# wangkenpu/rsrgan

Measured on AMD Instinct MI355X. Metric: GAN train frames/sec (G+D step), 257-dim LPS->40-dim MFCC, higher is better.
Workload: dtype f32

## Files before the change

### rsrgan_amd/csrc/kernels.h

```cpp
#pragma once
#include <hip/hip_runtime.h>
#include <stdint.h>

#include "switches.h"

namespace rsr {

constexpr int MAXJ = 8;

struct Place { int x0, nx, sb, se, nb, w; };
constexpr int JOBMAP_MAX = 768;
struct JobMap { int valid; unsigned char job[JOBMAP_MAX]; };
struct PlanItem { int ncol, nrow; double cost; int mult; };
int plan_places(int n, const PlanItem* items, Place* out);

enum { DYN_G_LR = 0, DYN_D_LR = 1, DYN_LAMBDA = 2, DYN_D_REAL = 3, DYN_D_FAKE = 4, DYN_L2 = 5, DYN_CLIP = 6,
       DYN_B1 = 7, DYN_B2 = 8, DYN_EPS = 9, DYN_EMA = 10, DYN_ADAM_LRT = 11, DYN_ADAM_LRT_D = 12, DYN_COUNT = 16 };

struct FwdGateJob {
  const float* x;
  const float* KxT;
  const float* m;
  const float* KhT;
  const float* Wsw;
// ... 100 lines not shown
  unsigned long long* gran;
  unsigned* ctl;
  float forget_bias;
  const float* dout_top;
  int ld_dout;
  float* dy;
  const float* fc_w;
  float* dtop;
  int ld_dy, ld_fcw, ld_dtop, fc_P;
  const float* fc_b;
  const float* noise;
  int xd_Ns, xd_row0;
  int Ns, row0;
  int nrt;
  float* dw_ws;
  unsigned* dw_flag;
  size_t dw_stride;
};
int dpersist_dw_grid(int nl, int N);
size_t dpersist_dw_stride(const DPersistArgs& a);
size_t dpersist_dw_flag_bytes(int nl, int N, int T);
bool dpersist_dw_supported(const DPersistArgs& a);
size_t dpersist_granule_bytes(int nl, int N, int T);
int dpersist_trail_grid(int nl, int N);
size_t dpersist_trail_lds_bytes();
bool dpersist_trail_supported(const DPersistArgs& a);
bool dpersist_supported(const DPersistArgs& a);
int dpersist_grid(int nl, int N);
size_t dpersist_lds_bytes();
void launch_dlstm_fwd(const DPersistArgs& a, hipStream_t s);
void launch_dlstm_fwd_t(const DPersistArgs& a, hipStream_t s);
void launch_dlstm_bwd(const DPersistArgs& a, hipStream_t s);
constexpr int GP_MAXL = 4;
constexpr int GP_ROWS = 32;
constexpr int GP_THREADS = 768;
struct GPersistLayer {
  const float *KxT, *KhT;
  const float *bias, *wi, *wf, *wo, *Wp;
  float *gates, *c, *h, *mst, *out;
  const float* in;
  float* dmt;
  int I, P, ldI, ldP, ldH;
  float* res_out;
};
struct GPersistArgs {
  GPersistLayer L[GP_MAXL];
  int nl, N, T, H;
  int NT, NC;
  const int* len;
  unsigned long long *gran1, *gran2;
  unsigned* ctl;
  float forget_bias;
  unsigned long long* gran3;
  const float* dout_top;
  int ld_dout;
  float* din0;
  int ld_din0;
  int res;
  int tags;
  int dout_trail;
  int fwd_trail;
  int ngl, grp0;
  int nrt;
  int sched;
  int carry;
};
constexpr int GP_TMAX = 2046;
bool gpersist_plan(GPersistArgs& a);
void gpersist_arm_bytes(void* p, size_t bytes, hipStream_t s);
extern thread_local int g_gemm_workers;
int gpersist_grid(const GPersistArgs& a);
int gpersist_dt_grid(const GPersistArgs& a, const DPersistArgs& d);
void launch_glstm_fwd_dt(const GPersistArgs& a, const DPersistArgs& d, hipStream_t s);
size_t dpersist_fwdt_lds_bytes();
void launch_glstm_bwd_dt(const GPersistArgs& a, const DPersistArgs& d, hipStream_t s);
size_t gpersist_lds_bytes();
int device_cu_count();
bool resident_probe(int grid, int threads, size_t lds_bytes);
size_t gpersist_gran1_bytes(const GPersistArgs& a);
size_t gpersist_gran2_bytes(const GPersistArgs& a);
size_t gpersist_gran3_bytes(const GPersistArgs& a);
void gpersist_arm(const GPersistArgs& a, hipStream_t s);
void launch_glstm_fwd(const GPersistArgs& a, hipStream_t s);
bool gpersist_np_plan(GPersistArgs& a, int nt_force = 0);
size_t gpersist_np_gran2_bytes(const GPersistArgs& a);
size_t gpersist_np_lds_bytes();
void launch_glstm_np_fwd(const GPersistArgs& a, hipStream_t s);
size_t gpersist_np_gran1_bytes(const GPersistArgs& a);
size_t gpersist_np_gran3_bytes(const GPersistArgs& a);
void gpersist_np_arm(const GPersistArgs& a, hipStream_t s);
void launch_glstm_np_bwd(const GPersistArgs& a, hipStream_t s);
void launch_glstm_bwd(const GPersistArgs& a, hipStream_t s);
extern long long g_chain_launches;
void launch_floor_chain(float* a, float* b, int n, int mode, hipStream_t s);

struct GemmRowMap { int rows_per; long long outer; long long inner; };
void launch_gemm_mapped(const float* A, int lda, const GemmRowMap& ma, const float* A2, int lda2, int M1, bool a_kc, const float* B, int ldb,
                        bool b_kc, float* C, int ldc, int M, int N, int K, const float* bias, int act, float alpha,
                        bool accumulate, hipStream_t s, float* ws, size_t ws_floats);
constexpr int GEMM16_MAXB = 4;
struct Gemm16Batch { const float* A[GEMM16_MAXB]; const float* A2[GEMM16_MAXB]; const float* B[GEMM16_MAXB]; float* C[GEMM16_MAXB]; int n; };
void launch_gemm16_batch(const Gemm16Batch& bt, int lda, int lda2, int M1, int ldb, int ldc, int M, int N, int K, bool accumulate,
                         hipStream_t s, float* ws, size_t ws_floats);
void launch_gemm2(const float* A, int lda, const float* A2, int lda2, int M1, bool a_kc, const float* B, int ldb, bool b_kc,
                  float* C, int ldc, int M, int N, int K, const float* bias, int act, float alpha, bool accumulate,
                  hipStream_t s, float* ws, size_t ws_floats);
constexpr int GEMM_MAXB = 4;
bool launch_gemm_batch(int nb, const float* const* A, int lda, const float* const* A2, int lda2, int M1, const float* const* B, int ldb,
                       float* const* C, int ldc, int M, int N, int K, bool accumulate, hipStream_t s, float* ws, size_t ws_floats);
void launch_gemm(const float* A, int lda, bool a_kc, const float* B, int ldb, bool b_kc,
                 float* C, int ldc, int M, int N, int K,
                 const float* bias, int act, float alpha, bool accumulate, hipStream_t s,
                 float* splitk_ws = nullptr, size_t splitk_ws_floats = 0);

struct StagePack { const float* src; float* dst; int D, ld; };
struct StageCopy { const void* src; void* dst; int n; };
struct StageJobs { StagePack pack[2]; StageCopy copy[4]; int B, T; int Bt; };
void launch_stage_inputs(const StageJobs& j, hipStream_t s);
void launch_pack_tm(const float* src_bm, float* dst_tm, int B, int T, int D, int ld, hipStream_t s);
void launch_unpack_bm(const float* src_tm, int ld, float* dst_bm, int B, int T, int D, hipStream_t s, int Bt = 0);
void launch_build_d_input(const float* lab_tm, const float* y_tm, const float* noise_r, const float* noise_f,
                          float* xd, int B, int T, int D, int ld, bool with_real, hipStream_t s);
void launch_add_noise_rows(const float* src_tm, const float* noise, float* dst, int B, int T, int D, int ld,
                           int Ns, int row0, hipStream_t s);
void launch_transpose(const float* src, int lds, float* dst, int ldd, int R, int C, hipStream_t s);
void launch_fill(float* p, size_t n, float v, hipStream_t s);
struct SwizzleJob { const float* src; float* dst; int ld, gates, H, C, c0, K1, I, P, kx, nct, nkb, blk_base; };
struct SwizzleList { int n; SwizzleJob j[24]; };
void launch_swizzle_many(SwizzleList& sl, hipStream_t s);
inline size_t swizzle_floats(int nct, int nkb) { return (size_t)nct * nkb * 256; }
struct TransposeJob { const float* src; float* dst; int lds, ldd, R, C, blk_base; };
struct TransposeList { int n; TransposeJob j[16]; };
void launch_transpose_many(TransposeList& tl, hipStream_t s);
size_t conv_prep_floats(int S, int fw, int C);
void launch_conv_prep(const float* F, int ldf_src, int S, int fw, int Cin, int Cout, bool flip, float* Ft, hipStream_t s);
bool conv_fwd_supported(int C, int N, int S, int W, int fw);
void launch_conv_fwd(const float* in, int ldc_in, int C, const float* Ft, const float* bias, bool relu, float* out, int ldc_out, int N,
                     int R, int S, int W, int fw, hipStream_t s,
                     const float* mask = nullptr );
bool conv_wgrad_supported(int C, int N, int S, int W, int fw);
size_t conv_wgrad_ws_floats(int C, int R, int S, int W, int fw);
void launch_conv_wgrad(const float* in, int ldc_in, int C, const float* d, int ldc_d, int N, float* dW, int ldw, float* ws, int R, int S,
                       int W, int fw, hipStream_t s,
                       float* db = nullptr );
void launch_im2col(const float* src, size_t row_stride, int ldc, int C, int S, int W, int kh, int kw, float* col, int ldk, size_t M,
                   hipStream_t s);
void launch_expand_c4(const float* src, int ld_src, int n, float* dst, size_t rows, hipStream_t s);
void launch_col2im(const float* dcol, int ldk, int C, int S, int W, int kh, int kw, float* dst, int ldc, size_t M, hipStream_t s);
struct GStateLayer { float *c, *mst; int H, P, ldP, off; };
struct GStateArgs { GStateLayer L[GP_MAXL]; int nl, SF, rows, dir; float* state; size_t slot; const int* mask; };
void launch_gstate(const GStateArgs& a, hipStream_t s);
struct ZeroList { int n; float* p[32]; unsigned len[32]; };
void launch_zero_many(const ZeroList& zl, hipStream_t s);
struct ColsumsBatch { const float* dz[4]; const float* cprev[4]; const float* ccur[4]; float* db[4]; float* dwi[4]; float* dwf[4]; float* dwo[4]; int n; };
void launch_lstm_colsums_batch(const ColsumsBatch& bt, int rows, int H, float* scratch, hipStream_t s);
void launch_lstm_colsums(const float* dz, const float* cprev, const float* ccur, float* db, float* dwi, float* dwf, float* dwo,
                         int rows, int H, float* scratch , hipStream_t s);
void launch_lrelu_bwd(const float* hval, float* d, size_t rows, int cols, int ld, float alpha, hipStream_t s);
void launch_dropout_fwd(float* y, size_t rows, int cols, int ld, unsigned long long key, unsigned thr, float keep, hipStream_t s);
void launch_dropout_bwd(const float* y, float* d, size_t rows, int cols, int ld, float keep, hipStream_t s);
void launch_colsum_tall(const float* a, int lda, float* out, int rows, int cols, float* scratch, size_t scratch_floats, hipStream_t s);

struct BnVars {
  float *beta, *gamma;
  float *mm, *mv, *rm, *rmw, *rs, *rsw;
};
constexpr int BN_STAT_ROWS = 6;
void launch_bn_forward(const float* z, int ldz, float* y, int ldy, int rows, int cols, const BnVars& v, float* stat, int ldc, bool training,
                       bool relu, float* scratch, size_t scratch_floats, hipStream_t s, int calls = 1);
void launch_bn_backward(float* dy, int ldd, const float* y, int ldy, const float* z, int ldz, int rows, int cols, const float* stat, int ldc,
                        float* dbeta, float* dgamma, bool accumulate, bool relu, float* sums, float* scratch, size_t scratch_floats,
                        hipStream_t s, int calls = 1);
void launch_bn_commit(int cols, const BnVars& v, const float* stat, int ldc, int times, hipStream_t s);
struct BnCommit { BnVars v; const float* stat; int cols, ldc, times0, times1; };
struct BnCommitList { int n; BnCommit e[24]; };
void launch_bn_commit_many(const BnCommitList& cl, hipStream_t s);
void launch_colsum(const float* a, int lda, const float* b, int ldb, float* out, int rows, int cols,
                   float* scratch , hipStream_t s);

constexpr int DH_MAXR = 64;
struct DHeadArgs {
  const float* top; int ldt; const float* w; int ldw; const float* b;
  float* logits; int ldl; float* dlogits; float* dout; int ldo; float* gw; float* gb;
  int T, Nd, n_real, dR; const float* t_real; const float* t_fake; float* loss3; float* part; int want_grads, want_wgrads;
  int Bp, Bt;
};
void launch_dhead(const DHeadArgs& a, hipStream_t s);
void launch_lsgan(const float* logits, int ldl, float* dlogits, int T, int Nd, int n_real,
                  const float* target_real, const float* target_fake, float* loss3, hipStream_t s,
                  bool clip_on = false, float clip_lo = 0.f, float clip_hi = 0.f, int Bp = 0, int Bt = 0);
void launch_build_joint(const float* x, int ldx, int off, int dim, const float* tail, int ldt, int Dt, float* joint, int ldj,
                        int row0, int R, hipStream_t s);
void launch_slice_cols(const float* src, int lds, int off, float* dst, int ldd, int R, int C, hipStream_t s);
void launch_mse(const float* y, const float* lab, int ld, float* dy, int rows, int D, const float* lambda,
                bool accumulate, float* loss_out, float* scratch , hipStream_t s, int Bp = 0, int Bt = 0);
void launch_g_total(float* l4 , const float* lambda, hipStream_t s);
void launch_copy_f(const float* src, float* dst, int n, hipStream_t s);

struct ChunkTable {
  const int* tensor;
  const int* off;
  const int* len;
  const int* t_first;
  const int* t_count;
  const int* t_l2;
  int n_chunks, n_tensors;
};
void launch_sumsq(const float* g, const ChunkTable& ct, float* partial, hipStream_t s);
void launch_dw_reduce(const float* ws, size_t stride, int ntiles, const long long* src, float* g, const ChunkTable& ct, float* partial, hipStream_t s);
void launch_l2(const float* w, float* g, const ChunkTable& ct, const float* l2_scale, float* partial, hipStream_t s);
void launch_l2_total(const float* partial, int n_chunks, const float* l2_scale, float* out, hipStream_t s);
void launch_apply_sgd(float* w, const float* g, float* ema, const ChunkTable& ct, const float* partial,
                      const float* dyn, hipStream_t s);
void launch_apply_adam(float* w, const float* g, float* m, float* v, float* ema, const ChunkTable& ct,
                       const float* partial, const float* dyn, hipStream_t s, int lrt_slot = DYN_ADAM_LRT);
void launch_adam_tick(float* dyn, int* t, double b1, double b2, hipStream_t s, int lr_slot = DYN_G_LR, int lrt_slot = DYN_ADAM_LRT);
void launch_pad_copy(const float* dense, float* padded, int rows, int cols, int ld, bool to_padded, hipStream_t s);

}
```

### rsrgan_amd/csrc/kernels.hip

```cpp
#include <algorithm>
#include <cstdlib>

#include "kernels.h"

namespace rsr {

typedef float f32x4 __attribute__((ext_vector_type(4)));

__device__ __forceinline__ float sigmoid_(float x) { return 1.0f / (1.0f + expf(-x)); }

#ifdef RSR_TRACE
__device__ unsigned long long g_trace[8192 * 16];
#define TR_BEGIN() do { if (threadIdx.x == 0 && blockIdx.x < 8192) { unsigned long long* t_ = g_trace + (size_t)blockIdx.x * 16; \
    t_[0] = __builtin_amdgcn_s_memrealtime(); t_[1] = __builtin_amdgcn_s_memtime(); \
    t_[14] = __builtin_amdgcn_s_getreg(4 | (0 << 6) | (31 << 11)); t_[15] = __builtin_amdgcn_s_getreg(20 | (0 << 6) | (3 << 11)); \
    for (int i_ = 2; i_ < 14; ++i_) t_[i_] = 0; } } while (0)
#define TR_ID(ptr) do { if (threadIdx.x == 0 && blockIdx.x < 8192) g_trace[(size_t)blockIdx.x * 16 + 12] = (unsigned long long)(size_t)(ptr); } while (0)
#define TR(i) do { if (threadIdx.x == 0 && blockIdx.x < 8192) g_trace[(size_t)blockIdx.x * 16 + (i)] = __builtin_amdgcn_s_memtime(); } while (0)
#define TR_END() do { if (threadIdx.x == 0 && blockIdx.x < 8192) { g_trace[(size_t)blockIdx.x * 16 + 9] = __builtin_amdgcn_s_memtime(); \
    g_trace[(size_t)blockIdx.x * 16 + 13] = __builtin_amdgcn_s_memrealtime(); } } while (0)
#else
#define TR_BEGIN() do { } while (0)
#define TR_ID(ptr) do { } while (0)
#define TR(i) do { } while (0)
#define TR_END() do { } while (0)
#endif

template <typename T>
__device__ __forceinline__ T* as_global(T* p) { return (T*)(__attribute__((address_space(1))) T*)(unsigned long long)p; }
#define RSR_G(f) J.f = as_global(J.f);
__device__ __forceinline__ unsigned long long splitmix64(unsigned long long x) {
  x += 0x9E3779B97F4A7C15ull;
  x = (x ^ (x >> 30)) * 0xBF58476D1CE4E5B9ull;
  x = (x ^ (x >> 27)) * 0x94D049BB133111EBull;
  return x ^ (x >> 31);
}
__device__ __forceinline__ unsigned long long drop_key(const DropSpec& d) {
  return splitmix64(splitmix64(d.seed ^ (*d.ctr * 0xD1342543DE82EF95ull)) + d.tag);
}
__device__ __forceinline__ bool drop_on(unsigned long long key, size_t idx, unsigned thr) { return (unsigned)(splitmix64(key + idx) >> 40) < thr; }
__device__ __forceinline__ void globalize(FwdGateJob& J) {
  RSR_G(x) RSR_G(KxT) RSR_G(m) RSR_G(KhT) RSR_G(Wsw) RSR_G(zx) RSR_G(bias) RSR_G(wf) RSR_G(wi) RSR_G(wo) RSR_G(c_prev) RSR_G(c_out) RSR_G(gates)
  RSR_G(h) RSR_G(len) RSR_G(np_m_out) RSR_G(np_out) RSR_G(np_res_in) RSR_G(np_res_out)
}
__device__ __forceinline__ void globalize(FwdProjJob& J) {
  RSR_G(h) RSR_G(WpT) RSR_G(WpT_sw) RSR_G(m_prev) RSR_G(m_out) RSR_G(out) RSR_G(res_in) RSR_G(res_out) RSR_G(len) RSR_G(bias) RSR_G(noise)
  J.drop.ctr = as_global(J.drop.ctr);
}
__device__ __forceinline__ void globalize(BwdAJob& J) {
  RSR_G(dout) RSR_G(dmst) RSR_G(Wp) RSR_G(Wp_sw) RSR_G(dmt) RSR_G(gates) RSR_G(c_prev) RSR_G(c_cur) RSR_G(wf) RSR_G(wi) RSR_G(wo) RSR_G(dc) RSR_G(len)
  J.drop.ctr = as_global(J.drop.ctr);
}
__device__ __forceinline__ void globalize(BwdBJob& J) { RSR_G(dz) RSR_G(K) RSR_G(Ksw) RSR_G(dx) RSR_G(dmst) RSR_G(len) RSR_G(ws) }
#undef RSR_G
template <typename JobT, int OFF>
__device__ __forceinline__ JobT pick_job(const JobT* j, const int& n_ref, const JobMap& map, int bid, int& lb) {
  constexpr int ND = (int)(sizeof(JobT) / 4);
  static_assert(sizeof(JobT) % 4 == 0 && ND <= 64 && OFF + 5 < ND, "job record must fit one dword per lane");
  const int lane = threadIdx.x & 63;
  const int li = lane < ND ? lane : 0;
  unsigned v[MAXJ];
#pragma unroll
  for (int q = 0; q < MAXJ; ++q) v[q] = reinterpret_cast<const unsigned*>(j + q)[li];
  const int x = bid & 7, sr = bid >> 3;
  unsigned vs = v[0];
  lb = -1;
  if (map.valid) {
    const int ji = map.job[min(bid, JOBMAP_MAX - 1)];
#pragma unroll
    for (int q = 1; q < MAXJ; ++q) vs = ji == q ? v[q] : vs;
    const int x0 = __builtin_amdgcn_readlane((int)vs, OFF), nx = __builtin_amdgcn_readlane((int)vs, OFF + 1);
    const int sb = __builtin_amdgcn_readlane((int)vs, OFF + 2);
    lb = ji == 0xFF ? -1 : (sr - sb) * nx + ((x - x0) & 7);
  } else {
    const int n = n_ref;
#pragma unroll
    for (int q = 0; q < MAXJ; ++q) {
      const int x0 = __builtin_amdgcn_readlane((int)v[q], OFF), nx = __builtin_amdgcn_readlane((int)v[q], OFF + 1);
      const int sb = __builtin_amdgcn_readlane((int)v[q], OFF + 2), se = __builtin_amdgcn_readlane((int)v[q], OFF + 3);
      const int nb = __builtin_amdgcn_readlane((int)v[q], OFF + 4);
      const int k = (x - x0) & 7;
      const int l = (sr - sb) * nx + k;
      const bool take = q < n && k < nx && sr >= sb && sr < se && l < nb;
      vs = take ? v[q] : vs;
      lb = take ? l : lb;
    }
  }
  union U { JobT j; unsigned d[ND]; __device__ U() {} } u;
#pragma unroll
  for (int i = 0; i < ND; ++i) u.d[i] = (unsigned)__builtin_amdgcn_readlane((int)vs, i);
  globalize(u.j);
  return u.j;
}
#define RSR_PICK(JobT, field, lb) pick_job<JobT, (int)(__builtin_offsetof(JobT, field) / 4)>(jobs.j, jobs.n, jobs.map, bid, lb)
#define RSR_PICK_M(JobT, field, mapf, lb) pick_job<JobT, (int)(__builtin_offsetof(JobT, field) / 4)>(jobs.j, jobs.n, jobs.mapf, bid, lb)

template <typename JobT>
__device__ __forceinline__ JobT load_job(const JobT* p) {
  constexpr int ND = (int)(sizeof(JobT) / 4);
  static_assert(sizeof(JobT) % 4 == 0 && ND <= 64, "job record must fit one dword per lane");
  const int lane = threadIdx.x & 63;
  const unsigned v = reinterpret_cast<const unsigned*>(p)[lane < ND ? lane : 0];
  union U { JobT j; unsigned d[ND]; __device__ U() {} } u;
#pragma unroll
  for (int i = 0; i < ND; ++i) u.d[i] = (unsigned)__builtin_amdgcn_readlane((int)v, i);
  globalize(u.j);
  return u.j;
}

__device__ __forceinline__ bool tile_of_block(int lb, int nblk_c, const Place& pl, int& cb, int& rb) {
  if (lb < 0) return false;
  rb = lb / pl.w;
  cb = lb - rb * pl.w;
  return cb < nblk_c;
}

template <int RT>
struct Seg {
  const float* a[RT];
  const float* w;
  const float* wt;
  int ld;
  int nkb;
  bool wok;
};

template <int RT, int CH, bool TILED>
__device__ __forceinline__ void load_chunk(float4 (&av)[CH][RT], float4 (&bv)[CH], const Seg<RT>& s, int j0, int je, int q) {
#pragma unroll
  for (int c = 0; c < CH; ++c) {
    const int j = j0 + c, jc = min(j, s.nkb - 1);
    const int k = jc * 16 + 4 * q, kc = min(k, s.ld - 4);
    const float4 b = TILED ? *reinterpret_cast<const float4*>(s.wt + (size_t)jc * 256) : *reinterpret_cast<const float4*>(s.w + kc);
    const bool ok = (j < je) && (k < s.ld) && (TILED || s.wok);
    bv[c] = make_float4(ok ? b.x : 0.f, ok ? b.y : 0.f, ok ? b.z : 0.f, ok ? b.w : 0.f);
#pragma unroll
    for (int i = 0; i < RT; ++i) av[c][i] = *reinterpret_cast<const float4*>(s.a[i] + kc);
  }
}
template <int RT, int CH>
__device__ __forceinline__ void mma_chunk(f32x4 (&acc)[RT], const float4 (&av)[CH][RT], const float4 (&bv)[CH]) {
#pragma unroll
  for (int c = 0; c < CH; ++c) {
#pragma unroll
    for (int i = 0; i < RT; ++i) acc[i] = __builtin_amdgcn_mfma_f32_16x16x4f32(av[c][i].x, bv[c].x, acc[i], 0, 0, 0);
#pragma unroll
    for (int i = 0; i < RT; ++i) acc[i] = __builtin_amdgcn_mfma_f32_16x16x4f32(av[c][i].y, bv[c].y, acc[i], 0, 0, 0);
#pragma unroll
    for (int i = 0; i < RT; ++i) acc[i] = __builtin_amdgcn_mfma_f32_16x16x4f32(av[c][i].z, bv[c].z, acc[i], 0, 0, 0);
#pragma unroll
    for (int i = 0; i < RT; ++i) acc[i] = __builtin_amdgcn_mfma_f32_16x16x4f32(av[c][i].w, bv[c].w, acc[i], 0, 0, 0);
  }
}
// ... 1014 lines not shown
    else *o = v[0];
  }
}
void launch_im2col(const float* src, size_t row_stride, int ldc, int C, int S, int W, int kh, int kw, float* col, int ldk, size_t M,
                   hipStream_t s) {
  if (C % 4 == 0 && ldc % 4 == 0) {
    const size_t total = M * (size_t)(ldk / 4);
    hipLaunchKernelGGL(k_im2col<4>, dim3((unsigned)std::min<size_t>((total + 255) / 256, 1u << 20)), dim3(256), 0, s, src, row_stride, ldc, C,
                       S, W, kh, kw, col, ldk, M);
  } else {
    const size_t total = M * (size_t)ldk;
    hipLaunchKernelGGL(k_im2col<1>, dim3((unsigned)std::min<size_t>((total + 255) / 256, 1u << 20)), dim3(256), 0, s, src, row_stride, ldc, C,
                       S, W, kh, kw, col, ldk, M);
  }
}
__global__ __launch_bounds__(256) void k_col2im(const float* __restrict__ dcol, int ldk, int C, int S, int W, int kh, int kw,
                                                float* __restrict__ dst, int ldc, size_t M) {
  const int nv = ldc / 4;
  const size_t total = M * (size_t)nv;
  const int pt = (kh - 1) / 2, pl = (kw - 1) / 2;
  for (size_t i = (size_t)blockIdx.x * blockDim.x + threadIdx.x; i < total; i += (size_t)gridDim.x * blockDim.x) {
    const size_t p = i / nv;
    const int c = (int)(i - p * nv) * 4;
    const int w = (int)(p % W);
    const size_t rh = p / W;
    const int h = (int)(rh % S);
    float4 acc = make_float4(0.f, 0.f, 0.f, 0.f);
    if (c < C) {
      for (int dh = 0; dh < kh; ++dh) {
        const int ho = h - dh + pt;
        if (ho < 0 || ho >= S) continue;
        for (int dw = 0; dw < kw; ++dw) {
          const int wo = w - dw + pl;
          if (wo < 0 || wo >= W) continue;
          const size_t po = (rh - h + ho) * W + wo;
          const float4 t = *reinterpret_cast<const float4*>(dcol + po * ldk + (size_t)(dh * kw + dw) * C + c);
          acc.x += t.x; acc.y += t.y; acc.z += t.z; acc.w += t.w;
        }
      }
    }
    *reinterpret_cast<float4*>(dst + p * ldc + c) = acc;
  }
}
__global__ void k_expand_c4(const float* __restrict__ src, int ld_src, int n, float4* __restrict__ dst, size_t total) {
  for (size_t i = (size_t)blockIdx.x * blockDim.x + threadIdx.x; i < total; i += (size_t)gridDim.x * blockDim.x) {
    const size_t r = i / n;
    dst[i] = make_float4(src[r * ld_src + (i - r * n)], 0.f, 0.f, 0.f);
  }
}
void launch_expand_c4(const float* src, int ld_src, int n, float* dst, size_t rows, hipStream_t s) {
  const size_t total = rows * (size_t)n;
  hipLaunchKernelGGL(k_expand_c4, dim3((unsigned)std::min<size_t>((total + 255) / 256, 1u << 20)), dim3(256), 0, s, src, ld_src, n,
                     reinterpret_cast<float4*>(dst), total);
}
void launch_col2im(const float* dcol, int ldk, int C, int S, int W, int kh, int kw, float* dst, int ldc, size_t M, hipStream_t s) {
  const size_t total = M * (size_t)(ldc / 4);
  hipLaunchKernelGGL(k_col2im, dim3((unsigned)std::min<size_t>((total + 255) / 256, 1u << 20)), dim3(256), 0, s, dcol, ldk, C, S, W, kh, kw,
                     dst, ldc, M);
}

__global__ void k_gstate(GStateArgs a) {
  const int row = blockIdx.x, tid = threadIdx.x;
  float* st = a.state + (size_t)row * a.SF;
  if (a.dir == 2) {
    if (a.mask && a.mask[row] == 0) return;
    for (int i = tid; i < a.SF; i += blockDim.x) st[i] = 0.f;
    return;
  }
  for (int l = 0; l < a.nl; ++l) {
    const GStateLayer L = a.L[l];
    float* c = L.c + (a.slot + row) * L.H;
    float* m = L.mst + (a.slot + row) * L.ldP;
    float* sc = st + L.off;
    float* sm = sc + L.H;
    if (a.dir == 0) {
      for (int i = tid; i < L.H; i += blockDim.x) c[i] = sc[i];
      for (int i = tid; i < L.ldP; i += blockDim.x) m[i] = i < L.P ? sm[i] : 0.f;
    } else {
      for (int i = tid; i < L.H; i += blockDim.x) sc[i] = c[i];
      for (int i = tid; i < L.P; i += blockDim.x) sm[i] = m[i];
    }
  }
}
void launch_gstate(const GStateArgs& a, hipStream_t s) {
  if (a.rows <= 0) return;
  hipLaunchKernelGGL(k_gstate, dim3(a.rows), dim3(256), 0, s, a);
}

__global__ void k_zero_many(ZeroList zl) {
  const int j = blockIdx.y;
  if (j >= zl.n) return;
  float* p = zl.p[j];
  const size_t n = zl.len[j];
  for (size_t i = (size_t)blockIdx.x * blockDim.x + threadIdx.x; i < n; i += (size_t)gridDim.x * blockDim.x) p[i] = 0.f;
}
void launch_zero_many(const ZeroList& zl, hipStream_t s) {
  if (zl.n == 0) return;
  hipLaunchKernelGGL(k_zero_many, dim3(32, zl.n), dim3(256), 0, s, zl);
}

__global__ void k_fill(float* p, size_t n, float v) {
  for (size_t i = (size_t)blockIdx.x * blockDim.x + threadIdx.x; i < n; i += (size_t)gridDim.x * blockDim.x) p[i] = v;
}
void launch_fill(float* p, size_t n, float v, hipStream_t s) {
  if (n == 0) return;
  const int blocks = (int)min((size_t)2048, (n + 255) / 256);
  hipLaunchKernelGGL(k_fill, dim3(blocks), dim3(256), 0, s, p, n, v);
}

__global__ void k_lrelu_bwd(const float* __restrict__ hval, float* __restrict__ d, size_t rows, int cols, int ld, float alpha) {
  const size_t total = rows * (size_t)cols;
  for (size_t i = (size_t)blockIdx.x * blockDim.x + threadIdx.x; i < total; i += (size_t)gridDim.x * blockDim.x) {
    const size_t r = i / cols; const int c = (int)(i % cols);
    const size_t o = r * ld + c;
    if (!(hval[o] > 0.f)) d[o] *= alpha;
  }
}
void launch_lrelu_bwd(const float* hval, float* d, size_t rows, int cols, int ld, float alpha, hipStream_t s) {
  const size_t total = rows * cols;
  const int blocks = (int)min((size_t)2048, (total + 255) / 256);
  hipLaunchKernelGGL(k_lrelu_bwd, dim3(blocks), dim3(256), 0, s, hval, d, rows, cols, ld, alpha);
}

__global__ void k_drop_tick(unsigned long long* ctr) { if (threadIdx.x == 0) *ctr += 1ull; }
void launch_drop_tick(unsigned long long* ctr, hipStream_t s) { hipLaunchKernelGGL(k_drop_tick, dim3(1), dim3(64), 0, s, ctr); }
__global__ __launch_bounds__(256) void k_dropout_fwd(float* __restrict__ y, size_t rows, int cols, int ld, unsigned long long key, unsigned thr,
                                                     float keep) {
  const size_t n = rows * (size_t)cols;
  for (size_t i = (size_t)blockIdx.x * 256 + threadIdx.x; i < n; i += (size_t)gridDim.x * 256) {
    const size_t r = i / cols;
    float* p = y + r * ld + (i - r * cols);
    const bool on = (unsigned)(splitmix64(key + i) >> 40) < thr;
    *p = on ? *p / keep : 0.f;
  }
}
void launch_dropout_fwd(float* y, size_t rows, int cols, int ld, unsigned long long key, unsigned thr, float keep, hipStream_t s) {
  const size_t n = rows * (size_t)cols;
  if (n == 0) return;
  hipLaunchKernelGGL(k_dropout_fwd, dim3((unsigned)std::min<size_t>((n + 255) / 256, 8192)), dim3(256), 0, s, y, rows, cols, ld, key, thr, keep);
}
__global__ __launch_bounds__(256) void k_dropout_bwd(const float* __restrict__ y, float* __restrict__ d, size_t rows, int cols, int ld, float keep) {
  const size_t n = rows * (size_t)cols;
  for (size_t i = (size_t)blockIdx.x * 256 + threadIdx.x; i < n; i += (size_t)gridDim.x * 256) {
    const size_t r = i / cols, o = r * ld + (i - r * cols);
    d[o] = y[o] > 0.f ? d[o] / keep : 0.f;
  }
}
void launch_dropout_bwd(const float* y, float* d, size_t rows, int cols, int ld, float keep, hipStream_t s) {
  const size_t n = rows * (size_t)cols;
  if (n == 0) return;
  hipLaunchKernelGGL(k_dropout_bwd, dim3((unsigned)std::min<size_t>((n + 255) / 256, 8192)), dim3(256), 0, s, y, d, rows, cols, ld, keep);
}

constexpr int CS_SLICES = 64;
__global__ __launch_bounds__(256) void k_colsum1(const float* __restrict__ a, int lda, const float* __restrict__ b, int ldb,
                                                 float* __restrict__ scratch, int rows, int cols) {
  __shared__ float red[4][64];
  const int c = blockIdx.x * 64 + (threadIdx.x & 63), rl = threadIdx.x >> 6;
  const int per = (rows + CS_SLICES - 1) / CS_SLICES;
  const int rbeg = blockIdx.y * per, rend = min(rows, rbeg + per);
  float s = 0.f;
  if (c < cols) {
    for (int r = rbeg + rl; r < rend; r += 4) {
      const float v = a[(size_t)r * lda + c];
      s += b ? v * b[(size_t)r * ldb + c] : v;
    }
  }
  red[rl][threadIdx.x & 63] = s;
  __syncthreads();
  if (rl == 0 && c < cols)
    scratch[(size_t)blockIdx.y * cols + c] = ((red[0][threadIdx.x] + red[1][threadIdx.x]) + red[2][threadIdx.x]) + red[3][threadIdx.x];
}
__global__ void k_colsum2(const float* __restrict__ scratch, float* __restrict__ out, int cols) {
  const int c = blockIdx.x * blockDim.x + threadIdx.x;
  if (c >= cols) return;
  float s = 0.f;
  for (int i = 0; i < CS_SLICES; ++i) s += scratch[(size_t)i * cols + c];
  out[c] = s;
}
__global__ __launch_bounds__(256) void k_colsum1_n(const float* __restrict__ a, int lda, float* __restrict__ scratch, int rows, int cols,
                                                   int per) {
  __shared__ float red[4][64];
  const int c = blockIdx.x * 64 + (threadIdx.x & 63), rl = threadIdx.x >> 6;
  const int rbeg = blockIdx.y * per, rend = min(rows, rbeg + per);
  float s = 0.f;
  if (c < cols) {
#pragma unroll 4
    for (int r = rbeg + rl; r < rend; r += 4) s += a[(size_t)r * lda + c];
  }
  red[rl][threadIdx.x & 63] = s;
  __syncthreads();
  if (rl == 0 && c < cols)
    scratch[(size_t)blockIdx.y * cols + c] = ((red[0][threadIdx.x] + red[1][threadIdx.x]) + red[2][threadIdx.x]) + red[3][threadIdx.x];
}
__global__ __launch_bounds__(256) void k_colsum2_n(const float* __restrict__ scratch, float* __restrict__ out, int cols, int slices) {
  __shared__ float red[4][64];
  const int c = blockIdx.x * 64 + (threadIdx.x & 63), g = threadIdx.x >> 6;
  float s = 0.f;
  if (c < cols) {
#pragma unroll 4
    for (int i = g; i < slices; i += 4) s += scratch[(size_t)i * cols + c];
  }
  red[g][threadIdx.x & 63] = s;
  __syncthreads();
  if (g == 0 && c < cols) out[c] = ((red[0][threadIdx.x] + red[1][threadIdx.x]) + red[2][threadIdx.x]) + red[3][threadIdx.x];
}
void launch_colsum_tall(const float* a, int lda, float* out, int rows, int cols, float* scratch, size_t scratch_floats, hipStream_t s) {
  int slices = (int)std::min<size_t>(512, scratch_floats / (size_t)std::max(cols, 1));
  slices = std::max(1, std::min(slices, (rows + 63) / 64));
  const int per = (rows + slices - 1) / slices;
  slices = (rows + per - 1) / per;
  hipLaunchKernelGGL(k_colsum1_n, dim3((cols + 63) / 64, slices), dim3(256), 0, s, a, lda, scratch, rows, cols, per);
  hipLaunchKernelGGL(k_colsum2_n, dim3((cols + 63) / 64), dim3(256), 0, s, scratch, out, cols, slices);
}

__global__ __launch_bounds__(256) void k_lstm_colsums1(const float* __restrict__ dz, const float* __restrict__ cprev,
                                                       const float* __restrict__ ccur, float* __restrict__ scratch, int rows, int H) {
  __shared__ float red[7][4][64];
  const int c = blockIdx.x * 64 + (threadIdx.x & 63), rl = threadIdx.x >> 6;
  const int per = (rows + CS_SLICES - 1) / CS_SLICES;
  const int rbeg = blockIdx.y * per, rend = min(rows, rbeg + per);
  float s[7] = {0.f, 0.f, 0.f, 0.f, 0.f, 0.f, 0.f};
  if (c < H) {
#pragma unroll 4
    for (int r = rbeg + rl; r < rend; r += 4) {
      const float* z = dz + (size_t)r * 4 * H + c;
      const float di = z[0], dj = z[H], df = z[2 * H], d_o = z[3 * H];
      const float cp = cprev[(size_t)r * H + c], cc = ccur[(size_t)r * H + c];
      s[0] += di; s[1] += dj; s[2] += df; s[3] += d_o; s[4] += di * cp; s[5] += df * cp; s[6] += d_o * cc;
    }
  }
#pragma unroll
  for (int k = 0; k < 7; ++k) red[k][rl][threadIdx.x & 63] = s[k];
  __syncthreads();
  if (rl == 0 && c < H) {
    const int x = threadIdx.x;
#pragma unroll
    for (int k = 0; k < 7; ++k)
      scratch[((size_t)blockIdx.y * 7 + k) * H + c] = ((red[k][0][x] + red[k][1][x]) + red[k][2][x]) + red[k][3][x];
  }
}
__global__ void k_lstm_colsums2(const float* __restrict__ scratch, float* __restrict__ db, float* __restrict__ dwi,
                                float* __restrict__ dwf, float* __restrict__ dwo, int H) {
  const int c = blockIdx.x * blockDim.x + threadIdx.x;
  if (c >= H) return;
  float s[7] = {0.f, 0.f, 0.f, 0.f, 0.f, 0.f, 0.f};
#pragma unroll 8
  for (int i = 0; i < CS_SLICES; ++i)
#pragma unroll
    for (int k = 0; k < 7; ++k) s[k] += scratch[((size_t)i * 7 + k) * H + c];
  db[c] = s[0]; db[H + c] = s[1]; db[2 * H + c] = s[2]; db[3 * H + c] = s[3];
  dwi[c] = s[4]; dwf[c] = s[5]; dwo[c] = s[6];
}
__global__ __launch_bounds__(256) void k_lstm_colsums1_b(const ColsumsBatch bt, float* __restrict__ scratch, int rows, int H) {
  __shared__ float red[7][4][64];
  const int p = blockIdx.z;
  const float* __restrict__ dz = bt.dz[p]; const float* __restrict__ cprev = bt.cprev[p]; const float* __restrict__ ccur = bt.ccur[p];
  scratch += (size_t)p * CS_SLICES * 7 * H;
  const int c = blockIdx.x * 64 + (threadIdx.x & 63), rl = threadIdx.x >> 6;
  const int per = (rows + CS_SLICES - 1) / CS_SLICES;
  const int rbeg = blockIdx.y * per, rend = min(rows, rbeg + per);
  float s[7] = {0.f, 0.f, 0.f, 0.f, 0.f, 0.f, 0.f};
  if (c < H) {
#pragma unroll 4
    for (int r = rbeg + rl; r < rend; r += 4) {
      const float* z = dz + (size_t)r * 4 * H + c;
      const float di = z[0], dj = z[H], df = z[2 * H], d_o = z[3 * H];
      const float cp = cprev[(size_t)r * H + c], cc = ccur[(size_t)r * H + c];
      s[0] += di; s[1] += dj; s[2] += df; s[3] += d_o; s[4] += di * cp; s[5] += df * cp; s[6] += d_o * cc;
    }
  }
#pragma unroll
  for (int k = 0; k < 7; ++k) red[k][rl][threadIdx.x & 63] = s[k];
  __syncthreads();
  if (rl == 0 && c < H) {
    const int x = threadIdx.x;
#pragma unroll
    for (int k = 0; k < 7; ++k)
      scratch[((size_t)blockIdx.y * 7 + k) * H + c] = ((red[k][0][x] + red[k][1][x]) + red[k][2][x]) + red[k][3][x];
  }
}
__global__ void k_lstm_colsums2_b(const float* __restrict__ scratch, const ColsumsBatch bt, int H) {
  const int p = blockIdx.y;
  scratch += (size_t)p * CS_SLICES * 7 * H;
  const int c = blockIdx.x * blockDim.x + threadIdx.x;
  if (c >= H) return;
  float s[7] = {0.f, 0.f, 0.f, 0.f, 0.f, 0.f, 0.f};
#pragma unroll 8
  for (int i = 0; i < CS_SLICES; ++i)
#pragma unroll
    for (int k = 0; k < 7; ++k) s[k] += scratch[((size_t)i * 7 + k) * H + c];
  float* db = bt.db[p];
  db[c] = s[0]; db[H + c] = s[1]; db[2 * H + c] = s[2]; db[3 * H + c] = s[3];
  bt.dwi[p][c] = s[4]; bt.dwf[p][c] = s[5]; bt.dwo[p][c] = s[6];
}
void launch_lstm_colsums_batch(const ColsumsBatch& bt, int rows, int H, float* scratch, hipStream_t s) {
  hipLaunchKernelGGL(k_lstm_colsums1_b, dim3((H + 63) / 64, CS_SLICES, bt.n), dim3(256), 0, s, bt, scratch, rows, H);
  hipLaunchKernelGGL(k_lstm_colsums2_b, dim3((H + 255) / 256, bt.n), dim3(256), 0, s, scratch, bt, H);
}
void launch_lstm_colsums(const float* dz, const float* cprev, const float* ccur, float* db, float* dwi, float* dwf, float* dwo,
                         int rows, int H, float* scratch, hipStream_t s) {
  hipLaunchKernelGGL(k_lstm_colsums1, dim3((H + 63) / 64, CS_SLICES), dim3(256), 0, s, dz, cprev, ccur, scratch, rows, H);
  hipLaunchKernelGGL(k_lstm_colsums2, dim3((H + 255) / 256), dim3(256), 0, s, scratch, db, dwi, dwf, dwo, H);
}

void launch_colsum(const float* a, int lda, const float* b, int ldb, float* out, int rows, int cols, float* scratch, hipStream_t s) {
  hipLaunchKernelGGL(k_colsum1, dim3((cols + 63) / 64, CS_SLICES), dim3(256), 0, s, a, lda, b, ldb, scratch, rows, cols);
  hipLaunchKernelGGL(k_colsum2, dim3((cols + 255) / 256), dim3(256), 0, s, scratch, out, cols);
}

__device__ __forceinline__ float block_sum_1024(float v, float* red) {
  for (int o = 32; o > 0; o >>= 1) v += __shfl_down(v, o, 64);
  const int w = threadIdx.x >> 6;
  if ((threadIdx.x & 63) == 0) red[w] = v;
  __syncthreads();
  float s = 0.f;
  const int nw = (blockDim.x + 63) >> 6;
  for (int i = 0; i < nw; ++i) s += red[i];
  __syncthreads();
  return s;
}

__global__ __launch_bounds__(1024) void k_lsgan(const float* __restrict__ logits, int ldl, float* __restrict__ dlogits,
                                                int T, int Nd, int n_real, const float* __restrict__ t_real,
                                                const float* __restrict__ t_fake, float* __restrict__ loss3,
                                                int clip_on, float clip_lo, float clip_hi, int Bp, int Bt) {
  __shared__ float red[16];
  const int rows = T * Nd;
  const float tr = *t_real, tf = *t_fake;
  const int nr_ = Bp > 0 ? n_real / Bp * Bt : n_real, nf_ = Bp > 0 ? (Nd - n_real) / Bp * Bt : Nd - n_real;
  const float cr = (float)T * (float)nr_, cf = (float)T * (float)nf_;
  float sr = 0.f, sf = 0.f;
  for (int r = threadIdx.x; r < rows; r += blockDim.x) {
    const bool real = (r % Nd) < n_real;
    const bool valid = Bp <= 0 || ((r % Nd) % Bp) < Bt;
    const float raw = logits[(size_t)r * ldl];
    const float val = clip_on ? fminf(fmaxf(raw, clip_lo), clip_hi) : raw;
    const float d = valid ? val - (real ? tr : tf) : 0.f;
    if (real) sr += d * d; else sf += d * d;
    if (dlogits) dlogits[(size_t)r * ldl] = (clip_on && (raw < clip_lo || raw > clip_hi)) ? 0.f : 2.f * d / (real ? cr : cf);
  }
  sr = block_sum_1024(sr, red);
  sf = block_sum_1024(sf, red);
  if (threadIdx.x == 0) {
    const float lr_ = n_real > 0 ? sr / cr : 0.f;
    const float lf_ = (Nd - n_real) > 0 ? sf / cf : 0.f;
    loss3[0] = lr_; loss3[1] = lf_; loss3[2] = lr_ + lf_;
  }
}
void launch_lsgan(const float* logits, int ldl, float* dlogits, int T, int Nd, int n_real,
                  const float* t_real, const float* t_fake, float* loss3, hipStream_t s, bool clip_on, float clip_lo, float clip_hi,
                  int Bp, int Bt) {
  hipLaunchKernelGGL(k_lsgan, dim3(1), dim3(1024), 0, s, logits, ldl, dlogits, T, Nd, n_real, t_real, t_fake, loss3,
                     clip_on ? 1 : 0, clip_lo, clip_hi, Bp, Bt);
}

__global__ __launch_bounds__(64) void k_dhead1(const DHeadArgs a) {
  __shared__ float wsh[DH_MAXR + 1];
  const int lane = threadIdx.x;
  const int rows = a.T * a.Nd, dR = a.dR;
  if (lane < dR) wsh[lane] = a.w[(size_t)lane * a.ldw];
  if (lane == 0) wsh[DH_MAXR] = a.b[0];
  __syncthreads();
  const int r = blockIdx.x * 64 + lane;
  const bool on = r < rows;
  const float tr = *a.t_real, tf = *a.t_fake;
  const int nr_ = a.Bp > 0 ? a.n_real / a.Bp * a.Bt : a.n_real, nf_ = a.Bp > 0 ? (a.Nd - a.n_real) / a.Bp * a.Bt : a.Nd - a.n_real;
  const float cr = (float)a.T * (float)nr_, cf = (float)a.T * (float)nf_;
  float x[DH_MAXR];
  float logit = wsh[DH_MAXR];
  const float* xr = a.top + (size_t)(on ? r : 0) * a.ldt;
#pragma unroll
  for (int c = 0; c < DH_MAXR; c += 4) {
    float4 v = make_float4(0.f, 0.f, 0.f, 0.f);
    if (c < dR) v = *reinterpret_cast<const float4*>(xr + c);
    x[c] = v.x; x[c + 1] = v.y; x[c + 2] = v.z; x[c + 3] = v.w;
  }
#pragma unroll
  for (int c = 0; c < DH_MAXR; ++c) if (c < dR) logit += x[c] * wsh[c];
  const bool real = on && (r % a.Nd) < a.n_real;
  const bool valid = a.Bp <= 0 || ((r % a.Nd) % a.Bp) < a.Bt;
  const float d = valid ? logit - (real ? tr : tf) : 0.f;
  float sr = (on && real) ? d * d : 0.f, sf = (on && !real) ? d * d : 0.f;
  const float dl = on ? 2.f * d / (real ? cr : cf) : 0.f;
  if (on) {
    a.logits[(size_t)r * a.ldl] = logit;
    if (a.want_grads) {
      a.dlogits[(size_t)r * a.ldl] = dl;
      float* o = a.dout + (size_t)r * a.ldo;
#pragma unroll
      for (int c = 0; c < DH_MAXR; c += 4)
        if (c < dR) *reinterpret_cast<float4*>(o + c) = make_float4(dl * wsh[c], dl * wsh[c + 1], dl * wsh[c + 2], dl * wsh[c + 3]);
    }
  }
  auto wsum = [&](float v) { for (int o = 32; o > 0; o >>= 1) v += __shfl_down(v, o, 64); return v; };
  float* part = a.part + (size_t)blockIdx.x * (DH_MAXR + 3);
  sr = wsum(sr); sf = wsum(sf);
  if (lane == 0) { part[0] = sr; part[1] = sf; }
  if (a.want_wgrads) {
    const float sd = wsum(dl);
    if (lane == 0) part[2] = sd;
#pragma unroll
    for (int c = 0; c < DH_MAXR; ++c)
      if (c < dR) { const float v = wsum(x[c] * dl); if (lane == 0) part[3 + c] = v; }
  }
}
__global__ __launch_bounds__(1024) void k_dhead2(const DHeadArgs a, int nblocks) {
  __shared__ float tot[DH_MAXR + 3];
  const int q = threadIdx.x >> 4, j = threadIdx.x & 15;
  const int nq = a.want_wgrads ? 3 + a.dR : 2;
  float s = 0.f;
  if (q < nq)
    for (int b = j; b < nblocks; b += 16) s += a.part[(size_t)b * (DH_MAXR + 3) + q];
  s += __shfl_xor(s, 8); s += __shfl_xor(s, 4); s += __shfl_xor(s, 2); s += __shfl_xor(s, 1);
  if (q < nq && j == 0) {
    tot[q] = s;
    if (a.want_wgrads) {
      if (q == 2) a.gb[0] = s;
      if (q >= 3) a.gw[(size_t)(q - 3) * a.ldw] = s;
    }
  }
  __syncthreads();
  if (threadIdx.x == 0) {
    const int nr_ = a.Bp > 0 ? a.n_real / a.Bp * a.Bt : a.n_real, nf_ = a.Bp > 0 ? (a.Nd - a.n_real) / a.Bp * a.Bt : a.Nd - a.n_real;
    const float cr = (float)a.T * (float)nr_, cf = (float)a.T * (float)nf_;
    const float lr_ = a.n_real > 0 ? tot[0] / cr : 0.f;
    const float lf_ = (a.Nd - a.n_real) > 0 ? tot[1] / cf : 0.f;
    a.loss3[0] = lr_; a.loss3[1] = lf_; a.loss3[2] = lr_ + lf_;
  }
}
void launch_dhead(const DHeadArgs& a, hipStream_t s) {
  const int rows = a.T * a.Nd, nb = (rows + 63) / 64;
  hipLaunchKernelGGL(k_dhead1, dim3(nb), dim3(64), 0, s, a);
  hipLaunchKernelGGL(k_dhead2, dim3(1), dim3(1024), 0, s, a, nb);
}

__global__ void k_build_joint(const float* __restrict__ x, int ldx, int off, int dim, const float* __restrict__ tail, int ldt, int Dt,
                              float* __restrict__ joint, int ldj, int row0, int R) {
  const int W = dim + Dt;
  const size_t total = (size_t)R * W;
  for (size_t i = (size_t)blockIdx.x * blockDim.x + threadIdx.x; i < total; i += (size_t)gridDim.x * blockDim.x) {
    const int r = (int)(i / W), c = (int)(i % W);
    joint[(size_t)(row0 + r) * ldj + c] = c < dim ? x[(size_t)r * ldx + off + c] : tail[(size_t)r * ldt + (c - dim)];
  }
}
void launch_build_joint(const float* x, int ldx, int off, int dim, const float* tail, int ldt, int Dt, float* joint, int ldj,
                        int row0, int R, hipStream_t s) {
  const size_t total = (size_t)R * (dim + Dt);
  const int blocks = (int)min((size_t)2048, (total + 255) / 256);
  hipLaunchKernelGGL(k_build_joint, dim3(blocks), dim3(256), 0, s, x, ldx, off, dim, tail, ldt, Dt, joint, ldj, row0, R);
}
__global__ void k_slice_cols(const float* __restrict__ src, int lds_, int off, float* __restrict__ dst, int ldd, int R, int C) {
  const size_t total = (size_t)R * C;
  for (size_t i = (size_t)blockIdx.x * blockDim.x + threadIdx.x; i < total; i += (size_t)gridDim.x * blockDim.x) {
    const int r = (int)(i / C), c = (int)(i % C);
    dst[(size_t)r * ldd + c] = src[(size_t)r * lds_ + off + c];
  }
}
void launch_slice_cols(const float* src, int lds_, int off, float* dst, int ldd, int R, int C, hipStream_t s) {
  const size_t total = (size_t)R * C;
  const int blocks = (int)min((size_t)2048, (total + 255) / 256);
  hipLaunchKernelGGL(k_slice_cols, dim3(blocks), dim3(256), 0, s, src, lds_, off, dst, ldd, R, C);
}

constexpr int MSE_BLOCKS = 256;
__global__ __launch_bounds__(256) void k_mse1(const float* __restrict__ y, const float* __restrict__ lab, int ld,
                                              float* __restrict__ dy, int rows, int D, const float* __restrict__ lambda,
                                              int accumulate, float* __restrict__ scratch, int Bp, int Bt) {
  __shared__ float red[16];
  const size_t total = (size_t)rows * D;
  const int rows_eff = Bp > 0 ? rows / Bp * Bt : rows;
  const float scale = dy ? (*lambda) / (float)rows_eff : 0.f;
  float s = 0.f;
  for (size_t i = (size_t)blockIdx.x * blockDim.x + threadIdx.x; i < total; i += (size_t)gridDim.x * blockDim.x) {
    const size_t r = i / D; const int c = (int)(i % D);
    const size_t o = r * ld + c;
    const bool valid = Bp <= 0 || (int)(r % Bp) < Bt;
    const float d = valid ? y[o] - lab[o] : 0.f;
    s += d * d;
    if (dy) dy[o] = (accumulate ? dy[o] : 0.f) + scale * d;
  }
  s = block_sum_1024(s, red);
  if (threadIdx.x == 0) scratch[blockIdx.x] = s;
}
__global__ void k_mse2(const float* __restrict__ scratch, int rows, float* __restrict__ out) {
  if (threadIdx.x == 0) {
    float s = 0.f;
    for (int i = 0; i < MSE_BLOCKS; ++i) s += scratch[i];
    *out = 0.5f * s / (float)rows;
  }
}
void launch_mse(const float* y, const float* lab, int ld, float* dy, int rows, int D, const float* lambda,
                bool accumulate, float* loss_out, float* scratch, hipStream_t s, int Bp, int Bt) {
  hipLaunchKernelGGL(k_mse1, dim3(MSE_BLOCKS), dim3(256), 0, s, y, lab, ld, dy, rows, D, lambda, accumulate ? 1 : 0, scratch, Bp, Bt);
  hipLaunchKernelGGL(k_mse2, dim3(1), dim3(64), 0, s, scratch, Bp > 0 ? rows / Bp * Bt : rows, loss_out);
}

__global__ void k_g_total(float* l4, const float* lambda) {
  if (threadIdx.x == 0) l4[3] = l4[0] + (*lambda) * l4[1] + l4[2];
}
void launch_g_total(float* l4, const float* lambda, hipStream_t s) {
  hipLaunchKernelGGL(k_g_total, dim3(1), dim3(64), 0, s, l4, lambda);
}
__global__ void k_copy_f(const float* src, float* dst, int n) {
  const int i = blockIdx.x * blockDim.x + threadIdx.x;
  if (i < n) dst[i] = src[i];
}
void launch_copy_f(const float* src, float* dst, int n, hipStream_t s) {
  hipLaunchKernelGGL(k_copy_f, dim3((n + 255) / 256), dim3(256), 0, s, src, dst, n);
}


__global__ __launch_bounds__(256) void k_sumsq(const float* __restrict__ g, ChunkTable ct, float* __restrict__ partial) {
  __shared__ float red[16];
  const int c = blockIdx.x;
  const float* p = g + ct.off[c];
  const int n = ct.len[c];
  float s = 0.f;
  for (int i = threadIdx.x * 4; i < n; i += 1024) {
    const float4 v = *reinterpret_cast<const float4*>(p + i);
    s += (v.x * v.x + v.y * v.y) + (v.z * v.z + v.w * v.w);
  }
  s = block_sum_1024(s, red);
  if (threadIdx.x == 0) partial[c] = s;
}
void launch_sumsq(const float* g, const ChunkTable& ct, float* partial, hipStream_t s) {
  hipLaunchKernelGGL(k_sumsq, dim3(ct.n_chunks), dim3(256), 0, s, g, ct, partial);
}

__global__ __launch_bounds__(256) void k_dw_reduce(const float* __restrict__ ws, size_t stride, int ntiles, const long long* __restrict__ src,
                                                   float* __restrict__ g, ChunkTable ct, float* __restrict__ partial) {
  __shared__ float red[16];
  const int c = blockIdx.x;
  const int t = ct.tensor[c];
  const int off = ct.off[c], n = ct.len[c];
  const long long so = src[t];
  float s = 0.f;
  if (so < 0) {
    for (int i = threadIdx.x * 4; i < n; i += 1024) {
      const float4 v = *reinterpret_cast<const float4*>(g + off + i);
      s += (v.x * v.x + v.y * v.y) + (v.z * v.z + v.w * v.w);
    }
  } else {
    const float* p = ws + so + (off - ct.off[ct.t_first[t]]);
    for (int i = threadIdx.x * 4; i < n; i += 1024) {
      float4 a = *reinterpret_cast<const float4*>(p + i);
      for (int r = 1; r < ntiles; ++r) {
        const float4 b = *reinterpret_cast<const float4*>(p + (size_t)r * stride + i);
        a.x += b.x; a.y += b.y; a.z += b.z; a.w += b.w;
      }
      *reinterpret_cast<float4*>(g + off + i) = a;
      s += (a.x * a.x + a.y * a.y) + (a.z * a.z + a.w * a.w);
    }
  }
  s = block_sum_1024(s, red);
  if (threadIdx.x == 0) partial[c] = s;
}
void launch_dw_reduce(const float* ws, size_t stride, int ntiles, const long long* src, float* g, const ChunkTable& ct, float* partial, hipStream_t s) {
  hipLaunchKernelGGL(k_dw_reduce, dim3(ct.n_chunks), dim3(256), 0, s, ws, stride, ntiles, src, g, ct, partial);
}

__global__ __launch_bounds__(256) void k_l2(const float* __restrict__ w, float* __restrict__ g, ChunkTable ct,
                                            const float* __restrict__ l2_scale, float* __restrict__ partial) {
  __shared__ float red[16];
  const int c = blockIdx.x;
  const bool on = ct.t_l2[ct.tensor[c]] != 0;
  const int off = ct.off[c], n = ct.len[c];
  const float sc = *l2_scale;
  float s = 0.f;
  if (on) {
    for (int i = threadIdx.x; i < n; i += 256) {
      const float v = w[off + i];
      s += v * v;
      g[off + i] += sc * v;
    }
  }
  s = block_sum_1024(s, red);
  if (threadIdx.x == 0) partial[c] = s;
}
void launch_l2(const float* w, float* g, const ChunkTable& ct, const float* l2_scale, float* partial, hipStream_t s) {
  hipLaunchKernelGGL(k_l2, dim3(ct.n_chunks), dim3(256), 0, s, w, g, ct, l2_scale, partial);
}
__global__ __launch_bounds__(1024) void k_l2_total(const float* __restrict__ partial, int n, const float* __restrict__ l2_scale, float* out) {
  __shared__ float red[16];
  float s = 0.f;
  for (int i = threadIdx.x; i < n; i += blockDim.x) s += partial[i];
  s = block_sum_1024(s, red);
  if (threadIdx.x == 0) *out = 0.5f * (*l2_scale) * s;
}
void launch_l2_total(const float* partial, int n, const float* l2_scale, float* out, hipStream_t s) {
  hipLaunchKernelGGL(k_l2_total, dim3(1), dim3(1024), 0, s, partial, n, l2_scale, out);
}

__device__ __forceinline__ float tensor_clip_scale(const ChunkTable& ct, const float* partial, int c, float clip, float* red) {
  const int t = ct.tensor[c];
  const int first = ct.t_first[t], cnt = ct.t_count[t];
  float s = 0.f;
  for (int i = threadIdx.x; i < cnt; i += blockDim.x) s += partial[first + i];
  s = block_sum_1024(s, red);
  if (!(clip > 0.f)) return 1.0f;
  const float inv = s > 0.f ? 1.0f / sqrtf(s) : __builtin_inff();
  return clip * fminf(inv, 1.0f / clip);
}

__global__ __launch_bounds__(256) void k_apply_sgd(float* __restrict__ w, const float* __restrict__ g, float* __restrict__ ema,
                                                   ChunkTable ct, const float* __restrict__ partial, const float* __restrict__ dyn) {
  __shared__ float red[16];
  const int c = blockIdx.x;
  const float scale = tensor_clip_scale(ct, partial, c, dyn[DYN_CLIP], red);
  const float lr = dyn[DYN_D_LR], dec = dyn[DYN_EMA];
  const int off = ct.off[c], n = ct.len[c];
  for (int i = threadIdx.x; i < n; i += 256) {
    const float nw = w[off + i] - lr * (g[off + i] * scale);
    w[off + i] = nw;
    if (ema) ema[off + i] = dec * ema[off + i] + (1.f - dec) * nw;
  }
}
void launch_apply_sgd(float* w, const float* g, float* ema, const ChunkTable& ct, const float* partial, const float* dyn, hipStream_t s) {
  hipLaunchKernelGGL(k_apply_sgd, dim3(ct.n_chunks), dim3(256), 0, s, w, g, ema, ct, partial, dyn);
}

__global__ __launch_bounds__(256) void k_apply_adam(float* __restrict__ w, const float* __restrict__ g, float* __restrict__ m,
                                                    float* __restrict__ v, float* __restrict__ ema, ChunkTable ct,
                                                    const float* __restrict__ partial, const float* __restrict__ dyn, int lrt_slot) {
  __shared__ float red[16];
  const int c = blockIdx.x;
  const float scale = tensor_clip_scale(ct, partial, c, dyn[DYN_CLIP], red);
  const float b1 = dyn[DYN_B1], b2 = dyn[DYN_B2], eps = dyn[DYN_EPS], lrt = dyn[lrt_slot], dec = dyn[DYN_EMA];
  const int off = ct.off[c], n = ct.len[c];
  for (int i = threadIdx.x; i < n; i += 256) {
    const float gg = g[off + i] * scale;
    const float mm = b1 * m[off + i] + (1.f - b1) * gg;
    const float vv = b2 * v[off + i] + (1.f - b2) * gg * gg;
    m[off + i] = mm; v[off + i] = vv;
    const float nw = w[off + i] - lrt * mm / (sqrtf(vv) + eps);
    w[off + i] = nw;
    if (ema) ema[off + i] = dec * ema[off + i] + (1.f - dec) * nw;
  }
}
void launch_apply_adam(float* w, const float* g, float* m, float* v, float* ema, const ChunkTable& ct,
                       const float* partial, const float* dyn, hipStream_t s, int lrt_slot) {
  hipLaunchKernelGGL(k_apply_adam, dim3(ct.n_chunks), dim3(256), 0, s, w, g, m, v, ema, ct, partial, dyn, lrt_slot);
}

__global__ void k_adam_tick(float* dyn, int* t, double b1, double b2, int lr_slot, int lrt_slot) {
  if (threadIdx.x == 0) {
    const int tt = *t + 1;
    *t = tt;
// ... 24 lines not shown
```

### rsrgan_amd/csrc/model.cpp

```cpp
#include "model.h"

#include <cmath>
#include <cstdarg>
#include <cstdio>
#include <cstdlib>
#include <cstring>
#include <random>

namespace rsr {

static thread_local char g_err[512] = "";
void set_error(const char* fmt, ...) {
  va_list ap;
  va_start(ap, fmt);
  vsnprintf(g_err, sizeof(g_err), fmt, ap);
  va_end(ap);
}
const char* get_error() { return g_err; }

#define HIPC(expr)                                                                   \
  do {                                                                               \
    hipError_t e_ = (expr);                                                          \
    if (e_ != hipSuccess) {                                                          \
      set_error("%s failed: %s (%s:%d)", #expr, hipGetErrorString(e_), __FILE__, __LINE__); \
      return RSRGAN_ERR_HIP;                                                         \
    }                                                                                \
  } while (0)

int ParamSet::add(const std::string& name, int rows, int cols, bool is_vector) {
  TensorDesc d;
  d.name = name;
  d.rows = rows; d.cols = cols; d.ld = pad4(cols);
  d.off = padded; d.dense_off = dense;
  d.l2 = name.find("bias") == std::string::npos;
  d.is_vector = is_vector;
  padded += ((int64_t)rows * d.ld + 63) / 64 * 64;
  dense += (int64_t)rows * cols;
  t.push_back(d);
  return (int)t.size() - 1;
}

static inline uint64_t seg_key(int seg, int T, unsigned bits) { return ((uint64_t)seg << 48) | ((uint64_t)(unsigned)T << 16) | (bits & 0xffffu); }
enum { SEG_D = 1, SEG_G_MAIN = 2, SEG_G_FCIN = 3, SEG_G_LAYER0 = 4 , SEG_G_L2 = 20, SEG_G_TAIL = 21, SEG_APPLY_D = 22, SEG_APPLY_G = 23, SEG_G_BATCH = 24, SEG_BNL = 25 };

template <class F>
void Model::run_seg(uint64_t key, hipStream_t s, F&& body) {
  if (!graphs_on() || s == nullptr) { body(); return; }
  if (graphs.size() > 96) drop_graphs();
  GraphSlot& g = graphs[key];
  if (g.exec) { if (hipGraphLaunch(g.exec, s) != hipSuccess) { (void)hipGetLastError(); g.exec = nullptr; g.uses = -1; body(); } return; }
  if (g.uses < 0) { body(); return; }
  if (g.uses++ == 0) { body(); return; }
  if (hipStreamBeginCapture(s, hipStreamCaptureModeThreadLocal) != hipSuccess) { (void)hipGetLastError(); g.uses = -1; body(); return; }
  body();
  hipGraph_t gr = nullptr;
  if (hipStreamEndCapture(s, &gr) != hipSuccess || !gr) {
    (void)hipGetLastError(); g.uses = -1;
    if (switch_now_graph_debug()) fprintf(stderr, "rsrgan: capture of segment %llx failed, eager from here on\n", (unsigned long long)key);
    body(); return;
  }
  hipGraphExec_t ex = nullptr;
  if (hipGraphInstantiate(&ex, gr, nullptr, nullptr, 0) != hipSuccess || !ex) { (void)hipGetLastError(); (void)hipGraphDestroy(gr); g.uses = -1; body(); return; }
  (void)hipGraphDestroy(gr);
  g.exec = ex;
  if (hipGraphLaunch(g.exec, s) != hipSuccess) { (void)hipGetLastError(); (void)hipGraphExecDestroy(g.exec); g.exec = nullptr; g.uses = -1; body(); }
}
void Model::drop_graphs() {
  for (auto& kv : graphs) if (kv.second.exec) (void)hipGraphExecDestroy(kv.second.exec);
  graphs.clear();
}
hipStream_t Model::enter(hipStream_t caller) {
  if (caller != nullptr || !main_s) return caller;
  (void)hipEventRecord(ev_in, caller);
  (void)hipStreamWaitEvent(main_s, ev_in, 0);
  return main_s;
}
void Model::leave(hipStream_t caller, hipStream_t work) {
  if (work == caller) return;
  (void)hipEventRecord(ev_out, work);
  (void)hipStreamWaitEvent(caller, ev_out, 0);
}
const float* Model::stage_noise(const float* src, float* buf, hipStream_t s) {
  if (!src) return nullptr;
  (void)hipMemcpyAsync(buf, src, (size_t)Bt * Dout * sizeof(float), hipMemcpyDeviceToDevice, s);
  return buf;
}

template <typename T>
T* Model::alloc(size_t n) {
  void* p = nullptr;
  if (n == 0) n = 1;
  if (hipMalloc(&p, n * sizeof(T)) != hipSuccess) return nullptr;
  (void)hipMemset(p, 0, n * sizeof(T));
  allocs.push_back(p);
  return reinterpret_cast<T*>(p);
}

static void add_lstm(ParamSet& ps, std::vector<LstmLayer>& out, const std::string& prefix, int I, int H, int proj) {
  LstmLayer L;
  const int P = proj > 0 ? proj : H;
  L.has_proj = proj > 0;
  L.I = I; L.H = H; L.P = P; L.ldI = pad4(I); L.ldP = pad4(P); L.ldH = pad4(H);
  L.tK = ps.add(prefix + "/kernel", I + P, 4 * H, false);
  L.tb = ps.add(prefix + "/bias", 1, 4 * H, true);
  L.twf = ps.add(prefix + "/w_f_diag", 1, H, true);
  L.twi = ps.add(prefix + "/w_i_diag", 1, H, true);
  L.two = ps.add(prefix + "/w_o_diag", 1, H, true);
  L.tWp = L.has_proj ? ps.add(prefix + "/projection/kernel", H, P, false) : -1;
  out.push_back(L);
}

static int build_chunks(Model& M, ParamSet& ps) {
  constexpr int CH = 4096;
  std::vector<int> tensor, off, len, tfirst, tcount, tl2;
  for (size_t i = 0; i < ps.t.size(); ++i) {
    const int64_t n = (int64_t)ps.t[i].rows * ps.t[i].ld;
    tfirst.push_back((int)tensor.size());
    int cnt = 0;
    for (int64_t o = 0; o < n; o += CH) {
      tensor.push_back((int)i);
      off.push_back((int)(ps.t[i].off + o));
      len.push_back((int)std::min<int64_t>(CH, n - o));
      ++cnt;
    }
    tcount.push_back(cnt);
    tl2.push_back(ps.t[i].l2 ? 1 : 0);
  }
  auto up = [&](const std::vector<int>& v) -> int* {
    int* d = M.alloc<int>(v.size());
    if (d && hipMemcpy(d, v.data(), v.size() * sizeof(int), hipMemcpyHostToDevice) != hipSuccess) d = nullptr;
    return d;
  };
  ps.ct.tensor = up(tensor); ps.ct.off = up(off); ps.ct.len = up(len);
  ps.ct.t_first = up(tfirst); ps.ct.t_count = up(tcount); ps.ct.t_l2 = up(tl2);
  ps.ct.n_chunks = (int)tensor.size();
  ps.ct.n_tensors = (int)ps.t.size();
  ps.partial = M.alloc<float>(tensor.size());
  return (ps.ct.tensor && ps.partial) ? 0 : -1;
}

static void alloc_stash(Model& M, LstmStash& S, const LstmLayer& L, int N, int T) {
  S.gates = M.alloc<float>((size_t)T * N * 4 * L.H);
  S.c = M.alloc<float>((size_t)(T + 1) * N * L.H);
  S.h = M.alloc<float>((size_t)T * N * L.ldH);
  S.mst = M.alloc<float>((size_t)(T + 1) * N * L.ldP);
  S.out = M.alloc<float>((size_t)T * N * L.ldP);
  S.dmt = M.alloc<float>((size_t)T * N * L.ldP);
  S.dc = M.alloc<float>((size_t)N * L.H);
  S.dmst = M.alloc<float>((size_t)N * L.ldP);
}

static hipError_t ctl_reset(unsigned* ctl) {
  const unsigned ctl0[DP_CTL_WORDS] = {1u, 0u, 0u, 0u};
  return hipMemcpy(ctl, ctl0, sizeof(ctl0), hipMemcpyHostToDevice);
}

int Model::init(const rsrgan_cfg& c, uint64_t seed) {
  cfg = c;
  B = Bt = c.batch_size; Tmax = c.max_frames; Din = c.input_dim; Dout = c.output_dim;
  ldDin = pad4(Din); ldDout = pad4(Dout);
  if (B <= 0 || Tmax <= 0 || Din <= 0 || Dout <= 0 || c.g_layers <= 0 || c.d_layers <= 0 || c.g_cells <= 0 ||
      c.d_cells <= 0 || (c.g_layers > MAXJ && !g_dnn()) || c.d_layers > MAXJ) {
    set_error("invalid sizes in rsrgan_cfg");
    return RSRGAN_ERR_INVALID;
  }
  if (c.d_type != RSRGAN_D_LSTM && c.d_type != RSRGAN_D_DNN) { set_error("Unrecognized D type %d", c.d_type); return RSRGAN_ERR_INVALID; }
  if (g_dnn() && !d_dnn()) { set_error("the frame-level generator (dnn) needs discriminator_dnn (models/gan.py:104)"); return RSRGAN_ERR_INVALID; }
  if (!g_dnn() && (c.g_proj < 0 || c.g_proj > 384)) { set_error("generator num_proj must be in [0, 384] (0 = num_proj=None)"); return RSRGAN_ERR_INVALID; }
  if (!d_dnn() && (c.d_proj < 0 || c.d_proj > 384)) { set_error("discriminator num_proj must be in [0, 384] (0 = num_proj=None)"); return RSRGAN_ERR_INVALID; }
  if (!g_dnn() && d_dnn() && c.d_joint_dim != 0) { set_error("discriminator_dnn on the sequence model is fed the target only (d_joint_dim must be 0)"); return RSRGAN_ERR_INVALID; }
  gR = c.g_proj > 0 ? c.g_proj : c.g_cells;
  dR = c.d_proj > 0 ? c.d_proj : c.d_cells;
  if (!g_dnn() && 2 * pad4(gR) > 1024) { set_error("generator layer input+state wider than 1024 floats is not supported by k_fwd_gates"); return RSRGAN_ERR_INVALID; }
  if (!d_dnn() && pad4(dR) + std::max(pad4(dR), pad4(c.output_dim)) > 1024) { set_error("discriminator layer too wide for k_fwd_gates"); return RSRGAN_ERR_INVALID; }
  if (d_dnn() && (c.d_joint_dim < 0 || c.d_joint_off < 0 || c.d_joint_off + c.d_joint_dim > Din)) { set_error("bad d_joint slice"); return RSRGAN_ERR_INVALID; }
  const int P = gR, H = c.g_cells;
  auto fc_name = [](const char* net, int i) { return std::string(net) + "/fully_connected" + (i == 0 ? "" : "_" + std::to_string(i)); };
  auto add_bn = [&](ParamSet& ps, const std::string& nm, int o, int (&tbn)[8]) {
    static const char* kBn[8] = {"beta", "gamma", "moving_mean", "moving_variance", "renorm_mean", "renorm_mean_weight", "renorm_stddev",
                                 "renorm_stddev_weight"};
    for (int k = 0; k < 8; ++k) {
      const bool scalar = k == 5 || k == 7;
      tbn[k] = ps.add(nm + "/BatchNorm/" + kBn[k], 1, scalar ? 1 : o, true);
      ps.t[tbn[k]].l2 = false;
      ps.t[tbn[k]].bias_init = (k == 1 || k == 3) ? 1.f : 0.f;
      ps.t[tbn[k]].trainable = k < 2;
    }
  };
  auto add_fc = [&](ParamSet& ps, std::vector<FcLayer>& out, const std::string& nm, int in, int o, bool bn = false) {
    FcLayer F; F.in = in; F.out = o; F.ld_in = pad4(in); F.ld_out = pad4(o);
    F.tW = ps.add(nm + "/weights", in, o, false);
    if (bn) {
      F.bn = true; F.tb = -1;
      add_bn(ps, nm, o, F.tbn);
    } else {
      F.tb = ps.add(nm + "/biases", 1, o, true);
    }
    out.push_back(F);
  };
  if (g_bnl()) { const int rc = bnl_check(c); if (rc) return rc; }
  if (bn_on() && !g_dnn()) {
    set_error("RSRGAN_FLAG_BATCH_NORM is built for the frame-level generators (dnn, rced) + discriminator_dnn only");
    return RSRGAN_ERR_INVALID;
  }
  if (bn_on()) {
    const int nbn = (c.g_type == RSRGAN_G_RCED ? 9 : c.g_layers) + (c.d_type == RSRGAN_D_DNN ? c.d_layers : 0);
    if (nbn > 24) { set_error("batch norm: %d normalised layers, at most 24 are supported", nbn); return RSRGAN_ERR_INVALID; }
  }
  if (c.g_type == RSRGAN_G_RCED) {
    static const int kNum[9] = {12, 16, 20, 24, 32, 24, 20, 16, 12}, kWidth[9] = {13, 11, 9, 7, 7, 7, 9, 11, 13};
    if (c.g_splice <= 0 || Din % c.g_splice) { set_error("R-CED: input_dim must be g_splice x frame width"); return RSRGAN_ERR_INVALID; }
    if (c.g_layers < 1 || c.g_layers > 9) { set_error("R-CED: g_layers must be in [1, 9]"); return RSRGAN_ERR_INVALID; }
    rcS = c.g_splice; rcW = Din / c.g_splice;
    int cin = 1;
    for (int l = 0; l < c.g_layers; ++l) {
      const int co = c.g_cells >= 32 ? kNum[l] : std::max(4, kNum[l] * c.g_cells / 32 / 4 * 4);
      ConvLayer L; L.fw = kWidth[l]; L.Cin = cin; L.Cout = co; L.K = rcS * L.fw * cin; L.ldK = pad4(L.K);
      L.ldCin = l == 0 ? 1 : pad4(cin); L.ldCout = pad4(co);
      const std::string nm = std::string("g_model/Conv") + (l == 0 ? "" : "_" + std::to_string(l));
      L.tW = G.add(nm + "/weights", L.K, co, false);
      if (bn_on()) { L.bn = true; L.tb = -1; add_bn(G, nm, co, L.tbn); }
      else L.tb = G.add(nm + "/biases", 1, co, true);
// ... 152 lines not shown
      }
    }
  }
  const int gmaxld = std::max(std::max(ldP, ldDin), ldDout);
  g_dA = alloc<float>(TB * gmaxld); g_dB = alloc<float>(TB * gmaxld); g_dC = alloc<float>(TB * gmaxld);
  const size_t TB2 = TB * 2;
  const int ldPd = d_dnn() ? 4 : pad4(dR);
  xd = alloc<float>(TB2 * ldDout); logits = alloc<float>(TB2 * 4); dlogits = alloc<float>(TB2 * 4);
  if (d_dnn()) {
    ldJ = pad4(c.d_joint_dim + Dout);
    if (c.d_joint_dim > 0) joint = alloc<float>(TB2 * ldJ);
    d_act.push_back(c.d_joint_dim > 0 ? joint : xd);
    for (size_t l = 0; l + 1 < dfc.size(); ++l) d_act.push_back(alloc<float>(TB2 * dfc[l].ld_out));
    d_act.push_back(logits);
    dy_buf = alloc<float>(TB * ldDout);
  }
  if (g_dnn() || d_dnn()) {
    int mx = std::max(ldJ, ldDin);
    for (auto& F : gfc) mx = std::max(mx, std::max(F.ld_in, F.ld_out));
    for (auto& F : dfc) mx = std::max(mx, std::max(F.ld_in, F.ld_out));
    fc_dA = alloc<float>(TB2 * mx); fc_dB = alloc<float>(TB2 * mx);
    if (bn_on()) {
      bn_sums = alloc<float>((size_t)2 * mx);
      for (auto& F : gfc) if (F.bn) { F.pre = alloc<float>(TB * F.ld_out); F.stat = alloc<float>((size_t)2 * BN_STAT_ROWS * F.ld_out); }
      for (auto& F : dfc) if (F.bn) { F.pre = alloc<float>(TB2 * F.ld_out); F.stat = alloc<float>((size_t)2 * BN_STAT_ROWS * F.ld_out); }
    }
  }
  adam_t_dev_d = alloc<int>(1);
  d_st.resize(dl.size());
  for (size_t l = 0; l < dl.size(); ++l) alloc_stash(*this, d_st[l], dl[l], 2 * B, Tmax);
  {
    bool ok = sw.dfold && !dl.empty();
    for (auto& L : dl) ok = ok && L.has_proj && L.H <= 288 && (L.ldH & 3) == 0;
    if (ok) {
      dl_fold.resize(dl.size()); dl_fold_K.resize(dl.size()); d_fold_st.resize(dl.size());
      for (size_t l = 0; l < dl.size(); ++l) {
        LstmLayer F = dl[l];
        F.has_proj = false; F.tWp = -1;
        F.I = l == 0 ? dl[0].I : dl[l - 1].H; F.ldI = l == 0 ? dl[0].ldI : dl[l - 1].ldH;
        F.P = dl[l].H; F.ldP = dl[l].ldH;
        F.KxT = F.KhT = F.WpT = nullptr; F.WpT_sw = F.Wp_sw = F.Kb_full = F.Kb_rec = nullptr;
        const int ncb = (F.H + 15) / 16;
        F.Wg_full = alloc<float>(swizzle_floats(4 * ncb, (F.ldI + F.ldP + 15) / 16));
        F.Wg_h = alloc<float>(swizzle_floats(4 * ncb, (F.ldP + 15) / 16));
        dl_fold_K[l] = alloc<float>((size_t)(F.I + F.H) * 4 * F.H);
        dl_fold[l] = F;
        LstmStash S = d_st[l];
        S.mst = alloc<float>((size_t)(Tmax + 1) * 2 * B * F.ldP);
        S.out = nullptr; S.dmt = nullptr; S.dmst = nullptr;
        d_fold_st[l] = S;
      }
    }
  }
  if (dp_live && !dl.empty() && dl.size() <= (size_t)DP_MAXL && B % 16 == 0) {
    const int nl_ = (int)dl.size();
    for (int rows : {2 * B, B}) {
      const int g_ = dpersist_grid(nl_, rows);
      if (g_ <= 128 && resident_probe(g_, 512, dpersist_lds_bytes())) { dp_max_grid = g_; break; }
    }
  }
  if (dp_max_grid > 0) {
    dp_gran_bytes = dpersist_granule_bytes((int)dl.size(), 2 * B, Tmax);
    dp_gran = (unsigned long long*)alloc<float>(dp_gran_bytes / sizeof(float));
    dp_ctl = (unsigned*)alloc<float>(16);
    HIPC(ctl_reset(dp_ctl));
    DPersistArgs pa{};
    pa.nl = (int)dl.size(); pa.N = 2 * B; pa.H = dl[0].H;
    for (size_t l = 0; l < dl.size(); ++l) { pa.L[l].I = dl[l].I; pa.L[l].P = dl[l].P; pa.L[l].ldP = dl[l].ldP; pa.L[l].ldI = dl[l].ldI; }
    bool shapes = switches().dw_inkernel && (dp_live & 2) && dpersist_dw_supported(pa) && !d_adam();
    for (auto& L : dl) shapes = shapes && L.has_proj && L.H == dl[0].H && L.ldH == dl[0].ldH;
    if (shapes && dpersist_grid(pa.nl, pa.N) == dp_max_grid) {
      const int nt = pa.N / 16;
      dw_stride = dpersist_dw_stride(pa);
      dw_ws = alloc<float>((size_t)pa.nl * nt * dw_stride);
      dw_flag = (unsigned*)alloc<float>(dpersist_dw_flag_bytes(pa.nl, pa.N, Tmax) / sizeof(float));
      std::vector<long long> src(D.t.size(), -1);
      const int IP = dl[0].I + dl[0].P, H4 = 4 * dl[0].H, H_ = dl[0].H;
      for (size_t l = 0; l < dl.size(); ++l) {
        const long long base = (long long)l * nt * (long long)dw_stride;
        src[dl[l].tK] = base; src[dl[l].tb] = base + (long long)IP * H4;
        const long long pp = base + (long long)(IP + 1) * H4;
        src[dl[l].twi] = pp; src[dl[l].twf] = pp + H_; src[dl[l].two] = pp + 2 * H_; src[dl[l].tWp] = pp + 3 * H_;
      }
      dw_src = (long long*)alloc<float>(src.size() * 2);
      if (dw_ws && dw_flag && dw_src) HIPC(hipMemcpy(dw_src, src.data(), src.size() * sizeof(long long), hipMemcpyHostToDevice));
      else dw_ws = nullptr;
    }
  }
  if (gp_live && !g_dnn() && !g_bnl()) {
    GPersistArgs ga{};
    gp_Tcap = std::min(Tmax, (int)GP_TMAX);
    gp_noproj = !gl.empty() && !gl[0].has_proj;
    if (gp_noproj) {
      bool fits = false;
      for (int nt : {2, 4}) {
        gp_np_nt = nt;
        if (gpersist_shape(ga, gp_Tcap) && resident_probe(gpersist_grid(ga), GP_THREADS, gpersist_np_lds_bytes())) { fits = true; break; }
      }
      if (!fits) gp_np_nt = 0;
      if (fits) {
        gp_gran2_bytes = gpersist_np_gran2_bytes(ga);
        gp_gran2 = (unsigned long long*)alloc<float>(gp_gran2_bytes / sizeof(float));
        gp_ctl = (unsigned*)alloc<float>(16);
        if (gp_np_nt == 2 && (gp_live & 2) && switches().gp_np_bwd) {
          gp_gran1 = (unsigned long long*)alloc<float>(gpersist_np_gran1_bytes(ga) / sizeof(float));
          gp_gran3 = (unsigned long long*)alloc<float>(gpersist_np_gran3_bytes(ga) / sizeof(float));
          if (!gp_gran1 || !gp_gran3) { gp_gran1 = gp_gran3 = nullptr; }
        }
        if (!gp_gran1) gp_gran1 = gp_gran2;
        if (gp_gran2 && gp_ctl) {
          HIPC(ctl_reset(gp_ctl));
          gpersist_rearm();
        } else { gp_gran1 = gp_gran2 = gp_gran3 = nullptr; gp_ctl = nullptr; }
      }
    } else if (gpersist_args(ga, gp_Tcap) && resident_probe(gpersist_grid(ga), GP_THREADS, gpersist_lds_bytes())) {
      gp_gran1 = (unsigned long long*)alloc<float>(gpersist_gran1_bytes(ga) / sizeof(float));
      gp_gran2_bytes = gpersist_gran2_bytes(ga);
      gp_gran2 = (unsigned long long*)alloc<float>(gp_gran2_bytes / sizeof(float));
      gp_ctl = (unsigned*)alloc<float>(16);
      bool bwd_ok = (gp_live & 2) != 0;
      for (auto& L : gl) bwd_ok = bwd_ok && L.P > 16;
      if (bwd_ok) gp_gran3 = (unsigned long long*)alloc<float>(gpersist_gran3_bytes(ga) / sizeof(float));
      if (gp_gran1 && gp_gran2 && gp_ctl) {
        HIPC(ctl_reset(gp_ctl));
        gpersist_rearm();
      } else { gp_gran1 = gp_gran2 = nullptr; gp_ctl = nullptr; }
    }
  }
  {
    GPersistArgs ga{};
    if (sw.trail && dp_gran && (dp_live & 2) && gp_gran1 && gp_gran3 && !gp_noproj && (gp_live & 2) && B % 32 == 0 && gpersist_args(ga, gp_Tcap))
      trail_fits = resident_probe(gpersist_grid(ga) + ((dpersist_trail_grid((int)dl.size(), B) + 7) & ~7), GP_THREADS,
                                  std::max(gpersist_lds_bytes(), dpersist_trail_lds_bytes()));
  }
  {
    lazy_sw = switches().lazy_swizzle && wavefront() && gp_gran1 && gp_gran3 && (gp_live & 3) == 3 && dp_gran && (dp_live & 3) == 3;
  }
  drop_ctr = (unsigned long long*)alloc<float>(4);
  HIPC(hipMemset(drop_ctr, 0, 16));
  const int dmaxld = std::max(ldPd, ldDout);
  d_dA = alloc<float>(TB2 * dmaxld); d_dB = alloc<float>(TB2 * dmaxld);
  len_dev = alloc<int>(2 * B);
  zeros = alloc<float>(64);
  noise_r_buf = alloc<float>((size_t)B * Dout); noise_f_buf = alloc<float>((size_t)B * Dout);
  if (hipStreamCreateWithFlags(&main_s, hipStreamNonBlocking) != hipSuccess) main_s = nullptr;
  if (main_s && (hipEventCreateWithFlags(&ev_in, hipEventDisableTiming) != hipSuccess ||
                 hipEventCreateWithFlags(&ev_out, hipEventDisableTiming) != hipSuccess)) { (void)hipStreamDestroy(main_s); main_s = nullptr; }
  dyn = alloc<float>(DYN_COUNT); adam_t_dev = alloc<int>(1);
  losses = alloc<float>(8); tmp3 = alloc<float>(4);
  size_t maxcols = 7 * (size_t)std::max(c.g_cells, c.d_cells);
  maxcols = std::max(maxcols, (size_t)Din + 4);
  maxcols = std::max(maxcols, (size_t)std::max(ldP, ldDin));
  scratch_floats = std::max<size_t>(4 * 64 * maxcols, 16384);
  scratch = alloc<float>(scratch_floats);
  scratch2 = alloc<float>(std::max<size_t>(4 * 64 * maxcols, 1024));
  g_fc_out_wT = g_dnn() ? nullptr : alloc<float>((size_t)Dout * ldP);
  if (hipStreamCreateWithFlags(&side, hipStreamNonBlocking) != hipSuccess) side = nullptr;
  if (hipEventCreateWithFlags(&ev_last, hipEventDisableTiming) != hipSuccess) ev_last = nullptr;
  {
    if (sw.dpipe > 0 && trail_fits && side && !d_dnn() && dp_max_grid >= dpersist_grid((int)dl.size(), B)) {
      const size_t gb = dpersist_granule_bytes((int)dl.size(), B, Tmax) / 2;
      dp_gran2 = (unsigned long long*)alloc<float>(gb / sizeof(float));
      dp_ctl2 = (unsigned*)alloc<float>(16);
      if (dp_gran2 && dp_ctl2 && hipEventCreateWithFlags(&ev_dfree, hipEventDisableTiming) == hipSuccess &&
          hipEventCreateWithFlags(&ev_real, hipEventDisableTiming) == hipSuccess) {
        HIPC(ctl_reset(dp_ctl2));
        dpipe = true;
      }
    }
  }
  if (side) {
    for (auto& e : ev_pool)
      if (hipEventCreateWithFlags(&e, hipEventDisableTiming) != hipSuccess) { side = nullptr; break; }
  }
  gemm_ws_floats = (size_t)32 << 20;
  gemm_ws = alloc<float>(gemm_ws_floats);
  if (!gemm_ws) gemm_ws_floats = 0;
  bwdb_ws_floats = (size_t)8 << 20;
  bwdb_ws = alloc<float>(bwdb_ws_floats);
  gemm_ws2 = alloc<float>(gemm_ws_floats ? gemm_ws_floats : 1);
  if (switches().dk_pad && !gl.empty() && gl[0].has_proj && gl[0].I % 4 != 0 && gl[0].ldI % 4 == 0 && gl.size() <= (size_t)GEMM_MAXB) {
    dk_tmp_per = (size_t)(gl[0].ldI + gl[0].P) * 4 * gl[0].H;
    dk_tmp = alloc<float>(dk_tmp_per * gl.size());
    if (!dk_tmp) dk_tmp_per = 0;
  }
  if (!gemm_ws2) side = nullptr;
  if (!side) dpipe = false;
  if (!scratch || !d_dB || !g_dB || !xd) { set_error("hipMalloc failed (activations)"); return RSRGAN_ERR_HIP; }

  std::mt19937_64 rng(seed);
  for (ParamSet* ps : {&G, &D}) {
    std::vector<float> host((size_t)ps->padded, 0.f);
    if (ps == &G && g_bnl()) bnl_init(host, seed);
    else for (auto& t : ps->t) {
      if (!t.l2) {
        if (t.bias_init != 0.f)
          for (int cc = 0; cc < t.cols; ++cc) host[(size_t)t.off + cc] = t.bias_init;
        continue;
      }
      const double fan_in = t.is_vector ? t.cols : t.rows, fan_out = t.xavier_fan_out > 0 ? t.xavier_fan_out : t.cols;
      const double lim = std::sqrt(6.0 / (fan_in + fan_out));
      std::uniform_real_distribution<double> u(-lim, lim);
      for (int r = 0; r < t.rows; ++r)
        for (int cc = 0; cc < t.cols; ++cc) host[(size_t)t.off + (size_t)r * t.ld + cc] = (float)u(rng);
    }
    HIPC(hipMemcpy(ps->w, host.data(), host.size() * sizeof(float), hipMemcpyHostToDevice));
    if (ps->ema) HIPC(hipMemcpy(ps->ema, host.data(), host.size() * sizeof(float), hipMemcpyHostToDevice));
  }
  scal[RSRGAN_G_LEARNING_RATE] = 8e-5; scal[RSRGAN_D_LEARNING_RATE] = 1e-3; scal[RSRGAN_MSE_LAMBDA] = 10.0;
  scal[RSRGAN_D_REAL] = 1.0; scal[RSRGAN_D_FAKE] = 0.0; scal[RSRGAN_L2_SCALE] = c.l2_scale;
  scal[RSRGAN_CLIP_NORM] = c.clip_norm; scal[RSRGAN_ADAM_STEP] = 0;
  float hdyn[DYN_COUNT] = {0};
  hdyn[DYN_G_LR] = 8e-5f; hdyn[DYN_D_LR] = 1e-3f; hdyn[DYN_LAMBDA] = 10.f; hdyn[DYN_D_REAL] = 1.f; hdyn[DYN_D_FAKE] = 0.f;
  hdyn[DYN_L2] = c.l2_scale; hdyn[DYN_CLIP] = c.clip_norm; hdyn[DYN_B1] = c.adam_beta1; hdyn[DYN_B2] = c.adam_beta2;
  hdyn[DYN_EPS] = c.adam_eps; hdyn[DYN_EMA] = c.ema_decay;
  HIPC(hipMemcpy(dyn, hdyn, sizeof(hdyn), hipMemcpyHostToDevice));
  refresh_transposes(RSRGAN_NET_G, nullptr);
  refresh_transposes(RSRGAN_NET_D, nullptr);
  { int rc = build_buckets(); if (rc) return rc; }
  HIPC(hipDeviceSynchronize());
  HIPC(hipGetLastError());
  return RSRGAN_OK;
}

void Model::destroy() {
  drop_graphs();
  if (main_s) {
    (void)hipStreamSynchronize(main_s);
    if (ev_in) (void)hipEventDestroy(ev_in);
    if (ev_out) (void)hipEventDestroy(ev_out);
    (void)hipStreamDestroy(main_s);
    main_s = nullptr;
  }
  if (side) {
    (void)hipStreamSynchronize(side);
    for (auto& e : ev_pool) if (e) (void)hipEventDestroy(e);
    (void)hipStreamDestroy(side);
    side = nullptr;
  }
  if (ev_last) { (void)hipEventDestroy(ev_last); ev_last = nullptr; ev_last_set = false; }
  if (ev_dfree) { (void)hipEventDestroy(ev_dfree); ev_dfree = nullptr; }
  if (ev_real) { (void)hipEventDestroy(ev_real); ev_real = nullptr; }
  dpipe = false;
  for (auto& v : gbk) { for (auto& b : v) if (b.ev) (void)hipEventDestroy(b.ev); v.clear(); }
  for (auto& e : prof_ev) if (e) (void)hipEventDestroy(e);
  prof_ev.clear();
  for (auto& e : prof_gp_ev) if (e) (void)hipEventDestroy(e);
  prof_gp_ev.clear();
  for (auto& e : prof_gb_ev) if (e) (void)hipEventDestroy(e);
  prof_gb_ev.clear();
  for (void* p : allocs) (void)hipFree(p);
  allocs.clear();
}

int Model::build_buckets() {
  auto range = [](const ParamSet& ps, int lo, int hi, GradBucket& b) {
    b.off = ps.t[lo].off;
    b.count = (hi + 1 < (int)ps.t.size() ? ps.t[hi + 1].off : ps.padded) - b.off;
  };
  auto whole = [](const ParamSet& ps, std::vector<GradBucket>& v) { GradBucket b; b.off = 0; b.count = ps.padded; v.assign(1, b); };
  whole(D, gbk[RSRGAN_NET_D]);
  whole(G, gbk[RSRGAN_NET_G]);
  if (!g_dnn() && wavefront()) {
    std::vector<GradBucket> v;
    bool ok = true;
    GradBucket b;
    range(G, g_fc_out_w, g_fc_out_b, b); ok = ok && g_fc_out_b == g_fc_out_w + 1; v.push_back(b);
    if (cfg.g_type == RSRGAN_G_LSTM) { range(G, g_fc_in_w, g_fc_in_b, b); ok = ok && g_fc_in_b == g_fc_in_w + 1; v.push_back(b); }
    for (auto& L : gl) {
      const int lo = L.tK, hi = L.has_proj ? L.tWp : L.two;
      ok = ok && L.tb > lo && L.tb < hi && L.twf > lo && L.twi > lo && L.two <= hi && hi - lo == (L.has_proj ? 5 : 4);
      range(G, lo, hi, b); v.push_back(b);
    }
    int64_t covered = 0;
    for (auto& x : v) covered += x.count;
    if (ok && covered == G.padded) gbk[RSRGAN_NET_G] = v;
  }
  for (auto& v : gbk)
    for (auto& b : v)
      if (hipEventCreateWithFlags(&b.ev, hipEventDisableTiming) != hipSuccess) { set_error("hipEventCreate failed"); return RSRGAN_ERR_HIP; }
  return RSRGAN_OK;
}
void Model::mark_bucket(int net, int i, hipStream_t s) {
  GradBucket& b = gbk[net][i];
  (void)hipEventRecord(b.ev, s);
  b.marked = true;
}
void Model::finish_buckets(int net, hipStream_t s) {
  for (auto& b : gbk[net]) {
    if (!b.marked) (void)hipEventRecord(b.ev, s);
    b.marked = false;
  }
}

void Model::refresh_transposes(int net, hipStream_t s) {
  const ParamSet& ps = net == RSRGAN_NET_G ? G : D;
  auto& layers = net == RSRGAN_NET_G ? gl : dl;
  TransposeList tl{};
  auto add = [&](const float* src, int lds_, float* dst, int ldd, int R, int C) {
    if (tl.n == 16) { launch_transpose_many(tl, s); tl.n = 0; }
    tl.j[tl.n++] = TransposeJob{src, dst, lds_, ldd, R, C, 0};
  };
  for (auto& L : layers) {
    const float* K = ps.W(L.tK);
    const int H4 = 4 * L.H;
    add(K, H4, L.KxT, L.ldI, L.I, H4);
    add(K + (size_t)L.I * H4, H4, L.KhT, L.ldP, L.P, H4);
    if (L.has_proj) add(ps.W(L.tWp), L.ldP, L.WpT, L.ldH, L.H, L.P);
// ... 826 lines not shown
      const int Lc = (int)ch.size(), off = offsets ? (*offsets)[c] : 0;
      for (int l = Lc - 1; l >= 0; --l) {
        const int t = T - 1 - (d - off - (Lc - 1 - l));
        if (t < 0 || t >= T) continue;
        if (aj.n == MAXJ) flush_a();
        BwdAJob& a = aj.j[aj.n++]; fill_bwd_a(a, ch[l], t); ab += bwd_a_blocks(ch[l].L->H, ch[l].N);
        ak = std::max(ak, kb16(ch[l].L->ldP));
      }
    }
    flush_a();
    for (size_t c = 0; c < chains.size(); ++c) {
      Chain& ch = chains[c];
      const int Lc = (int)ch.size(), off = offsets ? (*offsets)[c] : 0;
      for (int l = Lc - 1; l >= 0; --l) {
        const int t = T - 1 - (d - off - (Lc - 1 - l));
        if (t < 0 || t >= T) continue;
        const LayerRun& R = ch[l];
        if (bj.n == MAXJ) flush_b();
        BwdBJob& b = bj.j[bj.n++]; fill_bwd_b(b, R, t, R.din != nullptr); bb += job_blocks(b.nblk_c, R.N);
        bk = std::max(bk, kb16(4 * R.L->H));
      }
    }
    if (fcs)
      for (auto& F : *fcs) {
        const int t = T - 1 - (d - F.offset);
        if (t < 0 || t >= T) continue;
        if (bj.n == MAXJ) flush_b();
        BwdBJob& b = bj.j[bj.n++]; fill_fc_bwd(b, F, t); bb += job_blocks(b.nblk_c, F.N);
        bk = std::max(bk, kb16(F.ld_in));
      }
    flush_b();
    if (ovl) {
      for (size_t c = 0; c < chains.size(); ++c) {
        Chain& ch = chains[c];
        if (!ch[0].want_wgrads) continue;
        const int off = offsets ? (*offsets)[c] : 0, Lc = (int)ch.size();
        while (chunk_done[c] < nchunk && d >= (T - 1 - chunk_lo(chunk_done[c])) + off + Lc - 1) {
          const int cc = chunk_done[c]++;
          hipEvent_t ev = ev_pool[ev_next++ & 15];
          (void)hipEventRecord(ev, s);
          (void)hipStreamWaitEvent(side, ev, 0);
          for (auto& R : ch)
            if (R.want_wgrads) layer_wgrads_gemms(R, chunk_lo(cc), chunk_hi(cc), cc > 0, side);
        }
      }
    }
  }
  if (ovl) {
    for (auto& ch : chains)
      for (auto& R : ch)
        if (R.want_wgrads) layer_wgrads_colsums(R, T, side, scratch2);
    hipEvent_t ev = ev_pool[ev_next++ & 15];
    (void)hipEventRecord(ev, side);
    (void)hipStreamWaitEvent(s, ev, 0);
  } else if (!defer_wgrads) {
    for (auto& ch : chains)
      for (auto& R : ch)
        if (R.want_wgrads) layer_wgrads(R, T, s);
  }
}

int Model::prepare_batch(const float* x, const float* labels, const int32_t* lengths, int T, hipStream_t s, const float** nr,
                         const float** nf, hipStream_t early) {
  if (T <= 0 || T > Tmax) { set_error("T=%d outside (0, max_frames=%d]", T, Tmax); return RSRGAN_ERR_INVALID; }
  if (!x || (!lengths && !g_dnn())) { set_error("null input pointer"); return RSRGAN_ERR_INVALID; }
  StageJobs j{}; j.B = B; j.T = T; j.Bt = Bt;
  j.pack[0] = StagePack{x, x_tm, Din, ldDin};
  if (labels) j.pack[1] = StagePack{labels, lab_tm, Dout, ldDout};
  if (lengths) { j.copy[0] = StageCopy{lengths, len_dev, Bt}; j.copy[1] = StageCopy{lengths, len_dev + B, Bt}; }
  if (nr && *nr) { j.copy[2] = StageCopy{*nr, noise_r_buf, Bt * Dout}; *nr = noise_r_buf; }
  if (nf && *nf) { j.copy[3] = StageCopy{*nf, noise_f_buf, Bt * Dout}; *nf = noise_f_buf; }
  if (early) {
    StageJobs e{}; e.B = B; e.T = T; e.Bt = Bt;
    e.pack[1] = j.pack[1]; e.copy[0] = j.copy[0]; e.copy[1] = j.copy[1]; e.copy[2] = j.copy[2];
    j.pack[1] = StagePack{}; j.copy[0] = StageCopy{}; j.copy[1] = StageCopy{}; j.copy[2] = StageCopy{};
    (void)hipStreamWaitEvent(early, ev_dfree, 0);
    launch_stage_inputs(e, early);
  }
  launch_stage_inputs(j, s);
  cur_T = T;
  g_fwd_valid = false;
  return RSRGAN_OK;
}

Chain Model::g_chain(int T) {
  (void)T;
  Chain ch;
  const bool res = cfg.g_type == RSRGAN_G_RES_LSTM_L;
  for (size_t l = 0; l < gl.size(); ++l) {
    LayerRun R;
    R.ps = &G; R.L = &gl[l]; R.S = &g_st[l]; R.in = g_ins[l];
    R.N = B; R.Ns = B; R.row0 = 0; R.len = len_dev;
    R.zx_batched = (l == 0);
    R.carry = g_carry;
    if (res) { R.res_in = g_ins[l]; R.res_out = g_res[l]; }
    if (seq_drop_on()) R.drop = DropSpec{drop_ctr, drop_seed, (1ull << 40) | ((unsigned long long)l << 20), drop_thr(), keep_prob};
    ch.push_back(R);
  }
  return ch;
}

Chain Model::d_chain(int N, int Ns, int row0) {
  Chain ch;
  for (size_t l = 0; l < dl.size(); ++l) {
    LayerRun R;
    R.ps = &D; R.L = &dl[l]; R.S = &d_st[l]; R.in = l == 0 ? xd : d_st[l - 1].out;
    R.N = N; R.Ns = Ns; R.row0 = row0; R.len = len_dev + row0;
    R.zx_batched = false;
    ch.push_back(R);
  }
  return ch;
}

void Model::gstate_xfer(int dir, int T, int rows, const int* mask, hipStream_t s) {
  GStateArgs a{};
  a.nl = (int)gl.size(); a.SF = g_state_sf; a.rows = rows; a.dir = dir; a.state = g_state; a.slot = (size_t)T * B; a.mask = mask;
  int off = 0;
  for (size_t l = 0; l < gl.size(); ++l) {
    a.L[l] = GStateLayer{g_st[l].c, g_st[l].mst, gl[l].H, gl[l].P, gl[l].ldP, off};
    off += gl[l].H + gl[l].P;
  }
  launch_gstate(a, s);
}

void Model::g_forward_head(int T, hipStream_t s) {
  if (cfg.g_type == RSRGAN_G_LSTM) {
    const int P = gR, ldP = pad4(P);
    gemm(x_tm, ldDin, true, G.W(g_fc_in_w), ldP, false, g_h0, ldP, T * B, P, Din, G.W(g_fc_in_b), 1, cfg.lrelu_alpha, false, s);
  }
}
void Model::g_forward_tail(int T, hipStream_t s) {
  const int P = gR, ldP = pad4(P);
  gemm(g_ins[gl.size()], ldP, true, G.W(g_fc_out_w), ldDout, false, y_tm, ldDout, T * B, Dout, P, G.W(g_fc_out_b), 0, 0.f, false, s);
  g_fwd_valid = true;
}
void Model::g_forward(int T, hipStream_t s, Chain* extra) {
  if (g_dnn()) { bn_eval_call = false; g_frame_forward(T * B, s); g_fwd_valid = true; return; }
  if (g_bnl()) { bnl_forward(T, false, s); return; }
  g_forward_head(T, s);
  if (!extra && persist_forward_g(T, s)) { g_forward_tail(T, s); return; }
  std::vector<Chain> chains;
  chains.push_back(g_chain(T));
  if (extra) chains.push_back(*extra);
  rnn_forward(chains, T, s);
  g_forward_tail(T, s);
}

void Model::d_logits(int N, int T, hipStream_t s) {
  const int ldPd = pad4(dR);
  gemm(d_st[dl.size() - 1].out, ldPd, true, D.W(d_fc_w), 4, false, logits, 4, T * N, 1, dR, D.W(d_fc_b), 0, 0.f, false, s);
}

bool Model::d_head(int N, int T, int n_real, const float* t_real, const float* t_fake, float* loss3, bool want_grads, bool want_wgrads,
                   hipStream_t s) {
  const int ldPd = pad4(dR), nb = (T * N + 63) / 64;
  if (!switches().dhead || d_dnn() || dl.empty() || dR % 4 != 0 || dR + 3 > 64 ||
      (size_t)nb * (DH_MAXR + 3) > scratch_floats) return false;
  DHeadArgs a{};
  a.top = d_st[dl.size() - 1].out; a.ldt = ldPd; a.w = D.W(d_fc_w); a.ldw = 4; a.b = D.W(d_fc_b);
  a.logits = logits; a.ldl = 4; a.dlogits = dlogits; a.dout = d_dB; a.ldo = ldPd; a.gw = D.Gd(d_fc_w); a.gb = D.Gd(d_fc_b);
  a.T = T; a.Nd = N; a.n_real = n_real; a.dR = dR; a.t_real = t_real; a.t_fake = t_fake; a.loss3 = loss3; a.part = scratch;
  a.want_grads = want_grads ? 1 : 0; a.want_wgrads = want_wgrads ? 1 : 0;
  a.Bp = pad_Bp(); a.Bt = Bt;
  launch_dhead(a, s);
  return true;
}

void Model::d_backward_pass(int N, int T, bool want_wgrads, bool need_dx0, const float* dlog, hipStream_t s, bool head_done) {
  const int R = T * N;
  const int ldPd = pad4(dR);
  const size_t Ld = dl.size();
  const float* top = d_st[Ld - 1].out;
  if (want_wgrads && !head_done) {
    gemm(top, ldPd, false, dlog, 4, false, D.Gd(d_fc_w), 4, dR, 1, R, nullptr, 0, 0.f, false, s);
    launch_colsum(dlog, 4, nullptr, 0, D.Gd(d_fc_b), R, 1, scratch, s);
  }
  float* cur = d_dB;
  float* other = d_dA;
  if (!head_done) gemm(dlog, 4, true, D.W(d_fc_w), 4, true, cur, ldPd, R, dR, 1, nullptr, 0, 0.f, false, s);
  std::vector<Chain> chains(1, d_chain(N, N, 0));
  Chain& ch = chains[0];
  for (int l = (int)Ld - 1; l >= 0; --l) {
    ch[l].dout = cur;
    ch[l].din = (l > 0 || need_dx0) ? other : nullptr;
    ch[l].din_accumulate = false;
    ch[l].want_wgrads = want_wgrads;
    std::swap(cur, other);
  }
  if (!persist_backward(ch, T, s)) rnn_backward(chains, T, s);
  last_dx0 = cur;
}

void Model::g_backward_pass(int T, float* dy, hipStream_t s) {
  const int R = T * B;
  const int P = gR, ldP = pad4(P);
  const size_t Lg = gl.size();
  gemm(g_ins[Lg], ldP, false, dy, ldDout, false, G.Gd(g_fc_out_w), ldDout, P, Dout, R, nullptr, 0, 0.f, false, s);
  launch_colsum(dy, ldDout, nullptr, 0, G.Gd(g_fc_out_b), R, Dout, scratch, s);
  float* cur = g_dA;
  float* other = g_dB;
  gemm(dy, ldDout, true, G.W(g_fc_out_w), ldDout, true, cur, ldP, R, P, Dout, nullptr, 0, 0.f, false, s);
  std::vector<Chain> chains(1, g_chain(T));
  Chain& ch = chains[0];
  for (auto& r : ch) r.want_wgrads = true;
  if (cfg.g_type == RSRGAN_G_LSTM) {
    for (int l = (int)Lg - 1; l >= 0; --l) {
      ch[l].dout = cur; ch[l].din = other; ch[l].din_accumulate = false;
      std::swap(cur, other);
    }
    if (!persist_backward_g(ch, T, s)) rnn_backward(chains, T, s);
    launch_lrelu_bwd(g_h0, cur, (size_t)R, P, ldP, cfg.lrelu_alpha, s);
    gemm(x_tm, ldDin, false, cur, ldP, false, G.Gd(g_fc_in_w), ldP, Din, P, R, nullptr, 0, 0.f, false, s);
    launch_colsum(cur, ldP, nullptr, 0, G.Gd(g_fc_in_b), R, P, scratch, s);
  } else if (cfg.g_type == RSRGAN_G_RES_LSTM_L) {
    for (int l = (int)Lg - 1; l >= 0; --l) {
      ch[l].dout = cur; ch[l].din = l > 0 ? cur : nullptr; ch[l].din_accumulate = true;
    }
    if (!persist_backward_g(ch, T, s)) rnn_backward(chains, T, s);
  } else {
    for (int l = (int)Lg - 1; l >= 0; --l) {
      ch[l].dout = cur; ch[l].din = l > 0 ? other : nullptr; ch[l].din_accumulate = false;
      std::swap(cur, other);
    }
    if (!persist_backward_g(ch, T, s)) rnn_backward(chains, T, s);
  }
}

int Model::d_backward(const float* x, const float* labels, const int32_t* lengths, int T, const float* nr, const float* nf,
                      float* out_losses, bool want_grads, hipStream_t s) {
  if (!labels) { set_error("labels required"); return RSRGAN_ERR_INVALID; }
  if (supervised()) { set_error("RSRGAN_FLAG_SUPERVISED: the trainer graph has no discriminator step"); return RSRGAN_ERR_STATE; }
  if (g_dnn()) return dnn_d_backward(x, labels, T, out_losses, want_grads, s);
  if (d_dnn()) { nr = nullptr; nf = nullptr; }
  bn_eval_call = !want_grads;
  dfree_current = false;
  bool dsplit = false;
  if (dpipe && (!nr || sw.dpipe >= 2) && wavefront() && gp_fwd_on() && !d_dnn() && !seq_drop_on() && T > 0 && T <= Tmax) {
    Chain dchk = d_chain(B, 2 * B, B);
    dsplit = persist_forward_real(T, side, true) && persist_forward_g_trail(dchk, T, s, nf, true);
  }
  int rc = prepare_batch(x, labels, lengths, T, s, &nr, &nf, dsplit ? side : nullptr);
  if (rc) return rc;
  if (dsplit) {
    launch_add_noise_rows(lab_tm, nr, xd, B, T, Dout, ldDout, 2 * B, 0, side);
    (void)persist_forward_real(T, side);
    (void)hipEventRecord(ev_real, side);
    (void)hipStreamWaitEvent(s, ev_real, 0);
  }
  if (seq_drop_on()) launch_drop_tick(drop_ctr, s);
  const bool inl = fused_apply && switches().fused_seg && want_grads && !d_dnn() && graphs_on();
  const unsigned kbits = (want_grads ? 1u : 0u) | (nr ? 2u : 0u) | (nf ? 4u : 0u) | (inl ? 8u : 0u) | (dsplit ? 16u : 0u);
  run_seg(seg_key(SEG_D, T, kbits), s, [&]() {
  if (!dsplit) launch_add_noise_rows(lab_tm, nr, xd, B, T, Dout, ldDout, 2 * B, 0, s);
  bool g_done = false;
  if (dsplit) {
    g_forward_head(T, s);
    Chain dch = d_chain(B, 2 * B, B);
    g_done = persist_forward_g_trail(dch, T, s, nf);
  }
  if (!g_done && wavefront() && gp_fwd_on()) {
    g_forward_head(T, s);
    g_done = persist_forward_g(T, s);
    if (g_done) {
      g_forward_tail(T, s);
      launch_add_noise_rows(y_tm, nf, xd, B, T, Dout, ldDout, 2 * B, B, s);
      if (!d_dnn()) {
        std::vector<Chain> chains(1, d_chain(2 * B, 2 * B, 0));
        if (!persist_forward(chains[0], T, s)) rnn_forward(chains, T, s);
      }
    }
  }
  if (g_done) {
  } else if (wavefront()) {
    if (!gp_fwd_on()) g_forward_head(T, s);
    const int Lg = (int)gl.size(), ldP = pad4(gR);
    std::vector<Chain> chains{g_chain(T)};
    std::vector<int> offs{0};
    if (!d_dnn()) {
      chains.push_back(d_chain(B, 2 * B, 0)); offs.push_back(0);
      chains.push_back(d_chain(B, 2 * B, B)); offs.push_back(Lg + 1);
    }
    FcStage F;
    F.offset = Lg; F.N = B; F.K = gR; F.D = Dout;
    F.in = g_ins[Lg]; F.ld_in = ldP; F.WT = g_fc_out_wT; F.bias = G.W(g_fc_out_b); F.noise = nf;
    F.y = y_tm; F.ldy = ldDout; F.out2 = xd; F.ld2 = ldDout; F.Ns2 = 2 * B; F.row02 = B;
    std::vector<FcStage> fcs{F};
    rnn_forward(chains, T, s, &offs, &fcs);
  } else {
    g_forward(T, s);
    launch_add_noise_rows(y_tm, nf, xd, B, T, Dout, ldDout, 2 * B, B, s);
    if (!d_dnn()) {
      std::vector<Chain> chains(1, d_chain(2 * B, 2 * B, 0));
      rnn_forward(chains, T, s);
    }
  }
  if (d_dnn()) {
    d_dnn_forward_loss(T, 2 * B, B, want_grads, losses, s);
    if (want_grads) fc_backward(D, dfc, d_act, T * 2 * B, dlogits, true, false, s);
  } else {
    const bool head = d_head(2 * B, T, B, dyn + DYN_D_REAL, dyn + DYN_D_FAKE, losses, want_grads, want_grads, s);
    if (!head) {
      d_logits(2 * B, T, s);
      launch_lsgan(logits, 4, want_grads ? dlogits : nullptr, T, 2 * B, B, dyn + DYN_D_REAL, dyn + DYN_D_FAKE, losses, s, false, 0.f, 0.f, pad_Bp(), Bt);
    }
    if (want_grads) d_backward_pass(2 * B, T, true, false, dlogits, s, head);
  }
  if (inl) apply_body(RSRGAN_NET_D, s);
  });
  d_partial_fresh = false;
  g_fwd_valid = true;
  if (inl) apply_inlined |= 2;
  if (want_grads) { finish_buckets(RSRGAN_NET_D, s); d_grads_ready = true; }
  if (out_losses) launch_copy_f(losses, out_losses, 3, s);
  HIPC(hipGetLastError());
  return RSRGAN_OK;
}

int Model::g_backward(const float* x, const float* labels, const int32_t* lengths, int T, const float* nf,
                      float* out_losses, bool want_grads, bool reuse, hipStream_t s) {
  if (!labels) { set_error("labels required"); return RSRGAN_ERR_INVALID; }
  if (g_dnn()) return dnn_g_backward(x, labels, T, out_losses, want_grads, reuse, s);
  if (g_bnl()) return bnl_step(x, labels, lengths, T, out_losses, want_grads, s);
  bn_eval_call = !want_grads;
  dfree_current = false;
  if (seq_drop_on()) { reuse = false; launch_drop_tick(drop_ctr, s); }
  if (supervised()) {
    int rc = prepare_batch(x, labels, lengths, T, s);
    if (rc) return rc;
    g_forward(T, s);
    const bool l2s = !cfg.cross_validation && scal[RSRGAN_L2_SCALE] > 0.0;
    HIPC(hipMemsetAsync(losses + 3, 0, sizeof(float), s));
    if (want_grads) {
      float* dy = g_dC;
      launch_mse(y_tm, lab_tm, ldDout, dy, T * B, Dout, dyn + DYN_LAMBDA, false, losses + 4, scratch, s, pad_Bp(), Bt);
      g_backward_pass(T, dy, s);
      if (l2s) {
        launch_l2(G.w, G.g, G.ct, dyn + DYN_L2, G.partial, s);
        launch_l2_total(G.partial, G.ct.n_chunks, dyn + DYN_L2, losses + 5, s);
      }
      { finish_buckets(RSRGAN_NET_G, s); g_grads_ready = true; }
    } else {
      launch_mse(y_tm, lab_tm, ldDout, nullptr, T * B, Dout, dyn + DYN_LAMBDA, false, losses + 4, scratch, s, pad_Bp(), Bt);
    }
    if (!(want_grads && l2s)) HIPC(hipMemsetAsync(losses + 5, 0, sizeof(float), s));
    launch_g_total(losses + 3, dyn + DYN_LAMBDA, s);
    if (out_losses) launch_copy_f(losses + 3, out_losses, 4, s);
    HIPC(hipGetLastError());
    return RSRGAN_OK;
  }
  if (d_dnn()) nf = nullptr;
  if (reuse) {
    if (!g_fwd_valid || T != cur_T) { set_error("reuse_g_forward without a valid generator forward"); return RSRGAN_ERR_STATE; }
  } else {
    int rc = prepare_batch(x, labels, lengths, T, s);
    if (rc) return rc;
  }
  nf = stage_noise(nf, noise_f_buf, s);
  const bool l2_on = !cfg.cross_validation && scal[RSRGAN_L2_SCALE] > 0.0;
  const bool wave_bwd = want_grads && !d_dnn() && wavefront();
  const bool fused_seg = switches().fused_seg;
  const bool bucketed = wave_bwd && gbk[RSRGAN_NET_G].size() > 1 && !overlap() && !(fused_apply && fused_seg);
  const int R = T * B, Ld = (int)dl.size(), Lg = (int)gl.size();
  const int ldPd = pad4(dR), P = gR, ldP = pad4(P);
  float* dy = g_dB;
  float* bufA = g_dA; float* bufB = g_dC;
  std::vector<Chain> bw_chains;
  auto build_bw_chains = [&]() {
    Chain dch = d_chain(B, B, 0);
    float* cur = d_dB; float* other = d_dA;
    for (int l = Ld - 1; l >= 0; --l) {
      dch[l].dout = cur; dch[l].want_wgrads = false;
      if (l == 0) { dch[l].din = dy; dch[l].din_accumulate = true; }
      else { dch[l].din = other; dch[l].din_accumulate = false; std::swap(cur, other); }
    }
    Chain gch = g_chain(T);
    bufA = g_dA; bufB = g_dC;
    for (int l = Lg - 1; l >= 0; --l) {
      gch[l].want_wgrads = true;
      if (cfg.g_type == RSRGAN_G_RES_LSTM_L) {
        gch[l].dout = g_dA; gch[l].din = l > 0 ? g_dA : nullptr; gch[l].din_accumulate = true;
      } else {
        const bool need = cfg.g_type == RSRGAN_G_LSTM || l > 0;
        gch[l].dout = bufA; gch[l].din = need ? bufB : nullptr; gch[l].din_accumulate = false;
        std::swap(bufA, bufB);
      }
    }
    bw_chains = std::vector<Chain>{dch, gch};
  };
  if (wave_bwd) build_bw_chains();
  const bool fc_side_env = switches().wgrad_streams >= 2 && switches().fc_side;
  const bool fcs_inside = wave_bwd && !bucketed && side && fc_side_env && cfg.g_type == RSRGAN_G_LSTM && dl[0].ldI == ldDout &&
                          persist_backward_g(bw_chains[1], T, s, true);
  const bool inl = fused_apply && fused_seg && wave_bwd && !bucketed && graphs_on() && !(cfg.g_type == RSRGAN_G_LSTM && !fcs_inside);
  const unsigned kbits = (want_grads ? 1u : 0u) | (nf ? 2u : 0u) | (reuse ? 4u : 0u) | (l2_on ? 8u : 0u) | (bucketed ? 16u : 0u) | (inl ? 32u : 0u);
  auto tail_body = [&]() {
    if (want_grads && l2_on) {
      launch_l2(G.w, G.g, G.ct, dyn + DYN_L2, G.partial, s);
      launch_l2_total(G.partial, G.ct.n_chunks, dyn + DYN_L2, losses + 5, s);
    } else {
      (void)hipMemsetAsync(losses + 5, 0, sizeof(float), s);
    }
    launch_g_total(losses + 3, dyn + DYN_LAMBDA, s);
  };

  bool trail_plan = false;
  if (wave_bwd && want_grads && !d_dnn() && dl[0].ldI == ldDout && persist_backward_g(bw_chains[1], T, s, true)) {
    Chain dc0 = bw_chains[0];
    dc0[0].din = nullptr;
    trail_plan = persist_backward_trail(dc0, T, s, dy, ldDout, g_dA, ldP, true);
  }
  const bool gsplit = dpipe && trail_plan;
  auto bwd_rest = [&]() {
    const int ldP_ = pad4(gR);
    StreamFn pre, post;
    if (fcs_inside) {
      pre = [&](hipStream_t q) {
        gemm(g_ins[Lg], ldP_, false, dy, ldDout, false, G.Gd(g_fc_out_w), ldDout, gR, Dout, R, nullptr, 0, 0.f, false, q);
        launch_colsum(dy, ldDout, nullptr, 0, G.Gd(g_fc_out_b), R, Dout, (side && q == side) ? scratch2 : scratch, q);
      };
      post = [&](hipStream_t q) {
        launch_lrelu_bwd(g_h0, bufA, (size_t)R, gR, ldP_, cfg.lrelu_alpha, q);
        gemm(x_tm, ldDin, false, bufA, ldP_, false, G.Gd(g_fc_in_w), ldP_, Din, gR, R, nullptr, 0, 0.f, false, q);
        launch_colsum(bufA, ldP_, nullptr, 0, G.Gd(g_fc_in_b), R, gR, (side && q == side) ? scratch2 : scratch, q);
      };
    }
    const int saved_w = g_gemm_workers;
    g_gemm_workers = std::min(saved_w, switches().dpipe_w);
    defer_wgrads = bucketed;
    gp_phase = 2; persist_backward_g(bw_chains[1], T, s, false, pre, post); gp_phase = 0;
    defer_wgrads = false;
    if (!fcs_inside) {
      gemm(g_ins[Lg], ldP_, false, dy, ldDout, false, G.Gd(g_fc_out_w), ldDout, gR, Dout, R, nullptr, 0, 0.f, false, s);
      launch_colsum(dy, ldDout, nullptr, 0, G.Gd(g_fc_out_b), R, Dout, scratch, s);
    }
    g_gemm_workers = saved_w;
    if (inl) { tail_body(); apply_body(RSRGAN_NET_G, s); }
  };
  run_seg(seg_key(SEG_G_MAIN, T, kbits | (trail_plan ? 64u : 0u) | (gsplit ? 128u : 0u)), s, [&]() {
  if (trail_plan) gpersist_arm_bytes(g_dA, (size_t)T * B * ldP * sizeof(float), s);
  bool g_done = false;
  if (!reuse && !wavefront()) g_forward(T, s);
  bool d_trailed = false;
  if (!reuse && wavefront() && gp_fwd_on()) {
    g_forward_head(T, s);
    if (!d_dnn()) {
      Chain dch = d_chain(B, B, 0);
      g_done = d_trailed = persist_forward_g_trail(dch, T, s, nf);
    }
    if (!g_done) {
      g_done = persist_forward_g(T, s);
      if (g_done) g_forward_tail(T, s);
    }
  }
  if (d_trailed) {
  } else if (!reuse && wavefront() && !g_done) {
    if (!gp_fwd_on()) g_forward_head(T, s);
    std::vector<Chain> chains{g_chain(T)};
    std::vector<int> offs{0};
    if (!d_dnn()) { chains.push_back(d_chain(B, B, 0)); offs.push_back(Lg + 1); }
    FcStage F;
    F.offset = Lg; F.N = B; F.K = gR; F.D = Dout;
    F.in = g_ins[Lg]; F.ld_in = pad4(gR); F.WT = g_fc_out_wT; F.bias = G.W(g_fc_out_b); F.noise = nf;
    F.y = y_tm; F.ldy = ldDout; F.out2 = xd; F.ld2 = ldDout; F.Ns2 = B; F.row02 = 0;
    std::vector<FcStage> fcs{F};
    rnn_forward(chains, T, s, &offs, &fcs);
  } else {
    const bool direct = !nf && !d_dnn() && dl[0].ldI == ldDout;
    if (!direct) launch_add_noise_rows(y_tm, nf, xd, B, T, Dout, ldDout, B, 0, s);
    if (!d_dnn()) {
      std::vector<Chain> chains(1, d_chain(B, B, 0));
      if (direct) chains[0][0].in = y_tm;
      if (!persist_forward(chains[0], T, s) && !fold_forward(chains[0], T, s)) rnn_forward(chains, T, s);
    }
  }
  bool g_head = false;
  if (d_dnn()) {
    d_dnn_forward_loss(T, B, 0, want_grads, tmp3, s);
  } else {
    g_head = d_head(B, T, 0, dyn + DYN_D_REAL, dyn + DYN_D_REAL, tmp3, want_grads, false, s);
    if (!g_head) {
      d_logits(B, T, s);
      launch_lsgan(logits, 4, want_grads ? dlogits : nullptr, T, B, 0, dyn + DYN_D_REAL, dyn + DYN_D_REAL, tmp3, s, false, 0.f, 0.f, pad_Bp(), Bt);
    }
  }
  launch_copy_f(tmp3 + 1, losses + 3, 1, s);
  if (want_grads && d_dnn()) {
    float* dyd = fc_backward(D, dfc, d_act, T * B, dlogits, false, true, s);
    launch_mse(y_tm, lab_tm, ldDout, dyd, T * B, Dout, dyn + DYN_LAMBDA, true, losses + 4, scratch, s, pad_Bp(), Bt);
    g_backward_pass(T, dyd, s);
  } else if (wave_bwd) {
    if (!g_head) gemm(dlogits, 4, true, D.W(d_fc_w), 4, true, d_dB, ldPd, R, dR, 1, nullptr, 0, 0.f, false, s);
    launch_mse(y_tm, lab_tm, ldDout, dy, R, Dout, dyn + DYN_LAMBDA, false, losses + 4, scratch, s, pad_Bp(), Bt);
    FcStage F;
    F.offset = Ld; F.N = B; F.K = Dout; F.D = P;
    F.in = dy; F.ld_in = ldDout; F.WT = G.W(g_fc_out_w); F.y = g_dA; F.ldy = ldP; F.accumulate = false;
    std::vector<int> offs{0, Ld + 1};
    std::vector<FcStage> fcs{F};
    defer_wgrads = bucketed;
    if (dl[0].ldI == ldDout && persist_backward_g(bw_chains[1], T, s, true)) {
      std::vector<Chain> dc1(1, bw_chains[0]);
      dc1[0][0].din = nullptr;
      const bool trailed = trail_plan && persist_backward_trail(dc1[0], T, s, dy, ldDout, g_dA, ldP);
      if (!trailed) {
        if (!persist_backward(dc1[0], T, s)) rnn_backward(dc1, T, s);
        const int H4d = 4 * dl[0].H;
        gemm(d_st[0].gates, H4d, true, D.W(dl[0].tK), H4d, true, dy, ldDout, R, dl[0].I, H4d, nullptr, 0, 0.f, true, s);
        gemm(dy, ldDout, true, G.W(g_fc_out_w), ldDout, true, g_dA, ldP, R, P, Dout, nullptr, 0, 0.f, false, s);
      }
      gp_trail_next = trailed;
      StreamFn pre, post;
      if (fcs_inside) {
        pre = [&](hipStream_t q) {
          gemm(g_ins[Lg], ldP, false, dy, ldDout, false, G.Gd(g_fc_out_w), ldDout, P, Dout, R, nullptr, 0, 0.f, false, q);
          launch_colsum(dy, ldDout, nullptr, 0, G.Gd(g_fc_out_b), R, Dout, (side && q == side) ? scratch2 : scratch, q);
        };
        post = [&](hipStream_t q) {
          launch_lrelu_bwd(g_h0, bufA, (size_t)R, P, ldP, cfg.lrelu_alpha, q);
          gemm(x_tm, ldDin, false, bufA, ldP, false, G.Gd(g_fc_in_w), ldP, Din, P, R, nullptr, 0, 0.f, false, q);
          launch_colsum(bufA, ldP, nullptr, 0, G.Gd(g_fc_in_b), R, P, (side && q == side) ? scratch2 : scratch, q);
        };
      }
      if (gsplit) {
        gp_phase = 1; persist_backward_g(bw_chains[1], T, s, false, pre, post); gp_phase = 0;
        gp_trail_next = false;
        return;
      }
      persist_backward_g(bw_chains[1], T, s, false, pre, post);
      gp_trail_next = false;
    } else {
      rnn_backward(bw_chains, T, s, &offs, &fcs);
    }
    defer_wgrads = false;
    if (!fcs_inside) {
      gemm(g_ins[Lg], ldP, false, dy, ldDout, false, G.Gd(g_fc_out_w), ldDout, P, Dout, R, nullptr, 0, 0.f, false, s);
      launch_colsum(dy, ldDout, nullptr, 0, G.Gd(g_fc_out_b), R, Dout, scratch, s);
    }
  } else if (want_grads) {
    d_backward_pass(B, T, false, true, dlogits, s, g_head);
    float* dyd = last_dx0;
    launch_mse(y_tm, lab_tm, ldDout, dyd, T * B, Dout, dyn + DYN_LAMBDA, true, losses + 4, scratch, s, pad_Bp(), Bt);
    g_backward_pass(T, dyd, s);
  } else {
    launch_mse(y_tm, lab_tm, ldDout, nullptr, T * B, Dout, dyn + DYN_LAMBDA, false, losses + 4, scratch, s, pad_Bp(), Bt);
  }
  if (inl) { tail_body(); apply_body(RSRGAN_NET_G, s); }
  });
  if (gsplit) {
    defer_wgrads = false;
    (void)hipEventRecord(ev_dfree, s);
    dfree_inside = true; dfree_current = true;
    run_seg(seg_key(SEG_G_MAIN, T, kbits | 64u | 256u), s, bwd_rest);
  }
  if (inl) apply_inlined |= 1;
  if (!reuse) g_fwd_valid = true;
  if (wave_bwd) {
    int bi = 0;
    if (bucketed) mark_bucket(RSRGAN_NET_G, bi++, s);
    if (cfg.g_type == RSRGAN_G_LSTM && !fcs_inside) {
      run_seg(seg_key(SEG_G_FCIN, T, kbits), s, [&]() {
        launch_lrelu_bwd(g_h0, bufA, (size_t)R, P, ldP, cfg.lrelu_alpha, s);
        gemm(x_tm, ldDin, false, bufA, ldP, false, G.Gd(g_fc_in_w), ldP, Din, P, R, nullptr, 0, 0.f, false, s);
        launch_colsum(bufA, ldP, nullptr, 0, G.Gd(g_fc_in_b), R, P, scratch, s);
      });
      if (bucketed) mark_bucket(RSRGAN_NET_G, bi++, s);
    }
    if (bucketed) {
      bool dkd = false;
      const bool gb = batch_wgrads(bw_chains[1], T, s, false, &dkd, true);
      if (gb) run_seg(seg_key(SEG_G_BATCH, T, kbits), s, [&]() { bool d_ = false; (void)batch_wgrads(bw_chains[1], T, s, false, &d_); });
      int li = 0;
      for (auto& Rr : bw_chains[1]) {
        run_seg(seg_key(SEG_G_LAYER0 + li, T, kbits), s, [&]() { if (gb) layer_wgrads_gemms(Rr, 0, T, false, s, true, false); else layer_wgrads(Rr, T, s); });
        mark_bucket(RSRGAN_NET_G, bi++, s);
        ++li;
      }
    }
  }
  if (!inl) run_seg(seg_key(SEG_G_TAIL, T, kbits), s, tail_body);
  if (want_grads) {
    if (l2_on) for (auto& bk : gbk[RSRGAN_NET_G]) bk.marked = false;
    finish_buckets(RSRGAN_NET_G, s);
    g_grads_ready = true;
  }
  if (out_losses) launch_copy_f(losses + 3, out_losses, 4, s);
  HIPC(hipGetLastError());
  return RSRGAN_OK;
}

int Model::bnl_step(const float* x, const float* labels, const int32_t* lengths, int T, float* out_losses, bool want_grads, hipStream_t s) {
  if (want_grads && cfg.cross_validation) {
    set_error("g_type bnlstm: gradients of the cross_validation model (moving-statistics batch norm) are not built");
    return RSRGAN_ERR_INVALID;
  }
  int rc = prepare_batch(x, labels, lengths, T, s);
  if (rc) return rc;
  const bool l2s = want_grads && scal[RSRGAN_L2_SCALE] > 0.0;
  run_seg(seg_key(SEG_BNL, T, (want_grads ? 1u : 0u) | (l2s ? 2u : 0u)), s, [&]() {
    bnl_forward(T, want_grads, s);
    (void)hipMemsetAsync(losses + 3, 0, sizeof(float), s);
    float* dy = want_grads ? g_dC : nullptr;
    launch_mse(y_tm, lab_tm, ldDout, dy, T * B, Dout, dyn + DYN_LAMBDA, false, losses + 4, scratch, s, pad_Bp(), Bt);
    if (want_grads) bnl_backward(T, dy, s);
    if (l2s) {
      launch_l2(G.w, G.g, G.ct, dyn + DYN_L2, G.partial, s);
      launch_l2_total(G.partial, G.ct.n_chunks, dyn + DYN_L2, losses + 5, s);
    } else {
      (void)hipMemsetAsync(losses + 5, 0, sizeof(float), s);
    }
    launch_g_total(losses + 3, dyn + DYN_LAMBDA, s);
  });
  if (want_grads) { finish_buckets(RSRGAN_NET_G, s); g_grads_ready = true; }
  g_fwd_valid = false;
  if (out_losses) launch_copy_f(losses + 3, out_losses, 4, s);
  HIPC(hipGetLastError());
  return RSRGAN_OK;
}

void Model::apply_body(int net, hipStream_t s) {
  if (net == RSRGAN_NET_D) {
    if (!d_partial_fresh) launch_sumsq(D.g, D.ct, D.partial, s);
    d_partial_fresh = false;
    if (d_adam()) {
      launch_adam_tick(dyn, adam_t_dev_d, (double)cfg.adam_beta1, (double)cfg.adam_beta2, s, DYN_D_LR, DYN_ADAM_LRT_D);
      launch_apply_adam(D.w, D.g, D.m, D.v, D.ema, D.ct, D.partial, dyn, s, DYN_ADAM_LRT_D);
    } else {
      launch_apply_sgd(D.w, D.g, D.ema, D.ct, D.partial, dyn, s);
    }
    refresh_transposes(RSRGAN_NET_D, s);
  } else {
    launch_sumsq(G.g, G.ct, G.partial, s);
    launch_adam_tick(dyn, adam_t_dev, (double)cfg.adam_beta1, (double)cfg.adam_beta2, s);
    launch_apply_adam(G.w, G.g, G.m, G.v, G.ema, G.ct, G.partial, dyn, s);
    refresh_transposes(RSRGAN_NET_G, s);
  }
}

int Model::apply(int net, hipStream_t s) {
  if (net == RSRGAN_NET_D) {
    if (!d_grads_ready) { set_error("apply(D) without gradients"); return RSRGAN_ERR_STATE; }
    if (!(apply_inlined & 2)) run_seg(seg_key(SEG_APPLY_D, 0, 0), s, [&]() { apply_body(RSRGAN_NET_D, s); });
    apply_inlined &= ~2;
    if (d_adam()) scal[RSRGAN_ADAM_STEP_D] += 1;
    d_grads_ready = false;
  } else if (net == RSRGAN_NET_G) {
    if (!g_grads_ready) { set_error("apply(G) without gradients"); return RSRGAN_ERR_STATE; }
    if (!(apply_inlined & 1)) run_seg(seg_key(SEG_APPLY_G, 0, 0), s, [&]() { apply_body(RSRGAN_NET_G, s); });
    if (dfree_current) dfree_inside = true;
    apply_inlined &= ~1;
    scal[RSRGAN_ADAM_STEP] += 1;
    g_grads_ready = false;
    g_fwd_valid = false;
  } else {
    set_error("bad net %d", net);
    return RSRGAN_ERR_INVALID;
  }
  HIPC(hipGetLastError());
  return RSRGAN_OK;
}

}
```

### rsrgan_amd/csrc/model.h

```cpp
#pragma once
#include <hip/hip_runtime.h>
#include <stdint.h>
#include <string>
#include <unordered_map>
#include <functional>
#include <vector>

#include "../../include/rsrgan.h"
#include "kernels.h"

namespace rsr {

inline int pad4(int x) { return (x + 3) & ~3; }

struct TensorDesc {
  std::string name;
  int rows, cols, ld;
  int64_t off;
  int64_t dense_off;
  bool l2;
  bool trainable = true;
  bool is_vector;
  int xavier_fan_out = 0;
  float bias_init = 0.f;
// ... 104 lines not shown
void launch_bnl_ema(const BnlLayer& a, int T, float decay, hipStream_t s);
void launch_bnl_cell_bwd(const BnlLayer& a, int t, hipStream_t s);
void launch_bnl_dm(const BnlLayer& a, int t, hipStream_t s);
void launch_bnl_bn_in_bwd(const BnlLayer& a, float* dzx, int T, hipStream_t s);

struct Model {
  rsrgan_cfg cfg{};
  const HandleSwitches sw;
  int B = 0, Tmax = 0, Din = 0, Dout = 0, ldDin = 0, ldDout = 0;
  int Bt = 0;
  int pad_Bp() const { return Bt != B ? B : 0; }
  int gR = 0, dR = 0;
  ParamSet G, D;
  std::vector<LstmLayer> gl, dl;
  int g_fc_in_w = -1, g_fc_in_b = -1, g_fc_out_w = -1, g_fc_out_b = -1, d_fc_w = -1, d_fc_b = -1;

  float *x_tm = nullptr, *lab_tm = nullptr, *g_h0 = nullptr, *y_tm = nullptr;
  std::vector<float*> g_ins;
  std::vector<float*> g_res;
  std::vector<LstmStash> g_st;
  float *g_dA = nullptr, *g_dB = nullptr, *g_dC = nullptr;
  float *xd = nullptr, *logits = nullptr, *dlogits = nullptr;
  std::vector<LstmStash> d_st;
  float *d_dA = nullptr, *d_dB = nullptr, *last_dx0 = nullptr;
  int *len_dev = nullptr;
  float *zeros = nullptr;
  std::vector<LstmLayer> dl_fold;
  std::vector<float*> dl_fold_K;
  std::vector<LstmStash> d_fold_st;
  bool fold_forward(Chain& ch, int T, hipStream_t s);
  void refresh_fold(hipStream_t s);
  unsigned long long* dp_gran = nullptr;
  unsigned* dp_ctl = nullptr;
  size_t dp_gran_bytes = 0;
  int dp_live = sw.dpersist;
  bool persist_forward(Chain& ch, int T, hipStream_t s);
  bool persist_backward(Chain& ch, int T, hipStream_t s);
  bool persist_backward_trail(Chain& ch, int T, hipStream_t s, float* dy, int ld_dy, float* dtop, int ld_dtop, bool check_only = false);
  bool persist_forward_g_trail(Chain& ch, int T, hipStream_t s, const float* nf, bool check_only = false);
  bool dpipe = false;
  bool dfree_inside = false;
  bool dfree_current = false;
  int gp_phase = 0;
  hipEvent_t ev_dfree = nullptr, ev_real = nullptr;
  unsigned long long* dp_gran2 = nullptr;
  unsigned* dp_ctl2 = nullptr;
  bool persist_forward_real(int T, hipStream_t q, bool check_only = false);
  bool trail_fits = false;
  bool gp_trail_next = false;
  DPersistArgs dt_args{};
  unsigned long long *gp_gran1 = nullptr, *gp_gran2 = nullptr, *gp_gran3 = nullptr;
  unsigned* gp_ctl = nullptr;
  size_t gp_gran2_bytes = 0;
  int gp_live = sw.gpersist;
  int gp_Tcap = 0;
  float* dw_ws = nullptr; unsigned* dw_flag = nullptr; long long* dw_src = nullptr; size_t dw_stride = 0;
  bool d_partial_fresh = false;
  int dp_max_grid = 0;
  void persist_disable(int which);
  bool gp_fwd_on() const { return gp_gran1 && (gp_live & 1); }
  bool gpersist_shape(GPersistArgs& a, int T) const;
  int gp_np_nt = 0;
  bool gp_noproj = false;
  bool gpersist_args(GPersistArgs& a, int T) const;
  void gpersist_rearm();
  bool persist_forward_g(int T, hipStream_t s);
  float* g_state = nullptr;
  int g_state_sf = 0;
  bool g_carry = false;
  void gstate_xfer(int dir, int T, int rows, const int* mask, hipStream_t s);
  typedef std::function<void(hipStream_t)> StreamFn;
  bool persist_backward_g(Chain& ch, int T, hipStream_t s, bool check_only = false, const StreamFn& pre = nullptr, const StreamFn& post = nullptr);
  std::vector<FcLayer> gfc, dfc;
  std::vector<float*> g_act, d_act;
  float *fc_dA = nullptr, *fc_dB = nullptr, *joint = nullptr, *dy_buf = nullptr;
  int ldJ = 0;
  int *adam_t_dev_d = nullptr;
  bool g_dnn() const { return cfg.g_type == RSRGAN_G_DNN || cfg.g_type == RSRGAN_G_RCED; }
  bool g_rced() const { return cfg.g_type == RSRGAN_G_RCED; }
  std::vector<BnlCell> bnl;
  bool g_bnl() const { return cfg.g_type == RSRGAN_G_BNLSTM; }
  int bnl_check(const rsrgan_cfg& c) const;
  void bnl_params();
  int bnl_alloc();
  void bnl_init(std::vector<float>& host, uint64_t seed) const;
  BnlLayer bnl_args(int l, bool train) const;
  void bnl_forward(int T, bool train, hipStream_t s);
  void bnl_backward(int T, float* dy, hipStream_t s);
  int bnl_step(const float* x, const float* labels, const int32_t* lengths, int T, float* out_losses, bool want_grads, hipStream_t s);
  std::vector<ConvLayer> gconv;
  FcLayer rc_fc{};
  std::vector<float*> rc_act;
  float *rc_col = nullptr, *rc_dcol = nullptr, *rc_dA = nullptr, *rc_dB = nullptr;
  std::vector<float*> rc_cols;
  std::vector<float*> rc_ft_fwd, rc_ft_bwd;
  std::vector<char> rc_wgrad_implicit;
  float* rc_wg_ws = nullptr;
  float* rc_x4 = nullptr;
  bool rc_keep_cols = false;
  size_t scratch_floats = 0;
  int rcS = 0, rcW = 0;
  void g_frame_forward(int rows, hipStream_t s);
  void g_frame_backward(int rows, float* dy, hipStream_t s);
  void rced_forward(int rows, hipStream_t s);
  void rced_backward(int rows, float* dy, hipStream_t s);
  bool d_dnn() const { return cfg.d_type == RSRGAN_D_DNN; }
  bool d_adam() const { return g_dnn(); }
  void fc_forward(const ParamSet& ps, const std::vector<FcLayer>& L, const std::vector<float*>& act, int rows, hipStream_t s, int calls = 1,
                  int call0 = 0);
  float keep_prob = 1.f;
  uint64_t drop_seed = 0, drop_run = 0;
  bool drop_training() const {
    return g_dnn() && keep_prob < 1.f && !cfg.cross_validation && !bn_eval_call && scal[RSRGAN_L2_SCALE] > 0.0;
  }
  uint64_t drop_key(int net, int layer, int call) const;
  unsigned long long* drop_ctr = nullptr;
  bool seq_drop_on() const { return !g_dnn() && keep_prob < 1.f && !cfg.cross_validation && !bn_eval_call; }
  unsigned drop_thr() const { return (unsigned)((double)keep_prob * 16777216.0); }
  float* fc_backward(const ParamSet& ps, const std::vector<FcLayer>& L, const std::vector<float*>& act, int rows, float* dtop,
                     bool want_wgrads, bool want_din, hipStream_t s, int calls = 1, int row0 = 0, int call0 = 0);
  bool bn_on() const { return (cfg.flags & RSRGAN_FLAG_BATCH_NORM) != 0; }
  bool bn_eval_call = false;
  bool bn_training() const { return bn_on() && !cfg.cross_validation && !bn_eval_call; }
  BnVars bn_vars(const ParamSet& ps, const FcLayer& F) const;
  BnVars bn_vars(const ParamSet& ps, const int (&tbn)[8]) const;
  void bn_commit_stack(const ParamSet& ps, const std::vector<FcLayer>& L, int times0, int times1, BnCommitList& cl);
  float* bn_sums = nullptr;
  void d_dnn_forward_loss(int T, int Nd, int n_real, bool want_grads, float* loss3, hipStream_t s, int calls = 1, int call0 = 0);
  void bn_commit_run(bool with_d, hipStream_t s);
  int dnn_d_backward(const float* x, const float* labels, int T, float* out_losses, bool want_grads, hipStream_t s);
  int dnn_g_backward(const float* x, const float* labels, int T, float* out_losses, bool want_grads, bool reuse, hipStream_t s);

  float *dyn = nullptr;
  int *adam_t_dev = nullptr;
  float *losses = nullptr;
  float *tmp3 = nullptr;
  float *scratch = nullptr;
  double scal[RSRGAN_SCALAR_COUNT_] = {0};
  bool g_fwd_valid = false;
  int cur_T = 0;
  bool d_grads_ready = false, g_grads_ready = false;
  std::vector<void*> allocs;

  int init(const rsrgan_cfg& c, uint64_t seed);
  void destroy();

  int prepare_batch(const float* x, const float* labels, const int32_t* lengths, int T, hipStream_t s, const float** nr = nullptr,
                    const float** nf = nullptr, hipStream_t early = nullptr);
  void g_forward(int T, hipStream_t s, Chain* extra = nullptr);
  void g_forward_head(int T, hipStream_t s);
  void g_forward_tail(int T, hipStream_t s);
  void d_logits(int N, int T, hipStream_t s);
  void d_backward_pass(int N, int T, bool want_wgrads, bool need_dx0, const float* dlog, hipStream_t s, bool head_done = false);
  bool d_head(int N, int T, int n_real, const float* t_real, const float* t_fake, float* loss3, bool want_grads, bool want_wgrads, hipStream_t s);
  void g_backward_pass(int T, float* dy, hipStream_t s);
  int d_backward(const float* x, const float* labels, const int32_t* lengths, int T, const float* nr, const float* nf,
                 float* out_losses, bool want_grads, hipStream_t s);
  int g_backward(const float* x, const float* labels, const int32_t* lengths, int T, const float* nf,
                 float* out_losses, bool want_grads, bool reuse, hipStream_t s);
  int apply(int net, hipStream_t s);
  void apply_body(int net, hipStream_t s);
  int apply_inlined = 0;
  void refresh_transposes(int net, hipStream_t s);
  void refresh_swizzles(int net, hipStream_t s);
  bool lazy_sw = false;

  void rnn_forward(std::vector<Chain>& chains, int T, hipStream_t s, const std::vector<int>* offsets = nullptr,
                   const std::vector<FcStage>* fcs = nullptr);
  void rnn_backward(std::vector<Chain>& chains, int T, hipStream_t s, const std::vector<int>* offsets = nullptr,
                    const std::vector<FcStage>* fcs = nullptr);
  void layer_wgrads(const LayerRun& R, int T, hipStream_t s);
  void chain_wgrads(Chain& ch, int T, hipStream_t s, const StreamFn& between, const StreamFn& pre = nullptr, const StreamFn& post = nullptr);
  void layer_wgrads_gemms(const LayerRun& R, int t0, int t1, bool accumulate, hipStream_t s, bool do_dK = true, bool do_dWp = true);
  int trail_nrt() const;
  bool batch_wgrads(Chain& ch, int T, hipStream_t s, bool dK_too, bool* dK_done, bool check_only = false);
  void layer_wgrads_colsums(const LayerRun& R, int T, hipStream_t s, float* scr);
  hipStream_t side = nullptr;
  struct GradBucket { int64_t off = 0, count = 0; hipEvent_t ev = nullptr; bool marked = false; };
  std::vector<GradBucket> gbk[2];
  bool fused_apply = false;
  bool defer_wgrads = false;
  int build_buckets();
  void mark_bucket(int net, int i, hipStream_t s);
  void finish_buckets(int net, hipStream_t s);
  bool prof_on = false;
  std::vector<hipEvent_t> prof_ev;
  int prof_n = 0;
  double prof_flops = 0.0;
  std::vector<hipEvent_t> prof_gp_ev;
  int prof_gp_n = 0;
  double prof_gp_flops = 0.0;
  std::vector<hipEvent_t> prof_gb_ev;
  int prof_gb_n = 0;
  int prof_fdt_n = 0;
  int prof_cnt[9] = {};
  double prof_gb_flops = 0.0;
  void gates_launch(const FwdGateJobs& gj, int blocks, int kb, hipStream_t s);
  int gates_blocks(int H, int N) const;
  int proj_blocks(int P, int N) const;
  int bwd_a_blocks(int H, int N) const;
  void run_bwd_b_splitk(BwdBJobs& bj, hipStream_t s);
  hipEvent_t ev_pool[16] = {};
  int ev_next = 0;
  float* gemm_ws2 = nullptr;
  float* dk_tmp = nullptr;
  size_t dk_tmp_per = 0;
  float* scratch2 = nullptr;
  bool overlap() const { return side != nullptr && (cfg.flags & RSRGAN_FLAG_OVERLAP) != 0; }
  Chain g_chain(int T);
  Chain d_chain(int N, int Ns, int row0);
  void gemm(const float* A, int lda, bool a_kc, const float* B, int ldb, bool b_kc, float* C, int ldc, int M, int N,
            int K, const float* bias, int act, float alpha, bool accumulate, hipStream_t s);
  bool supervised() const { return (cfg.flags & RSRGAN_FLAG_SUPERVISED) != 0; }
  bool wavefront() const { return (cfg.flags & RSRGAN_FLAG_WAVEFRONT) != 0; }
  float* g_fc_out_wT = nullptr;
  float* bwdb_ws = nullptr;
  size_t bwdb_ws_floats = 0;
  bool bwd_b_splitk_ok(const BwdBJobs& jobs) const;
  float* gemm_ws = nullptr;
  size_t gemm_ws_floats = 0;

  struct GraphSlot { int uses = 0; hipGraphExec_t exec = nullptr; };
  std::unordered_map<uint64_t, GraphSlot> graphs;
  hipStream_t main_s = nullptr;
  hipEvent_t ev_in = nullptr, ev_out = nullptr;
  hipEvent_t ev_last = nullptr; bool ev_last_set = false;
  float *noise_r_buf = nullptr, *noise_f_buf = nullptr;
  bool graphs_on() const { return (cfg.flags & RSRGAN_FLAG_GRAPH) != 0 && wavefront() && !overlap() && !prof_on && !g_dnn() && sw.graphs; }
  template <class F> void run_seg(uint64_t key, hipStream_t s, F&& body);
  void drop_graphs();
  hipStream_t enter(hipStream_t caller);
  void leave(hipStream_t caller, hipStream_t work);
  const float* stage_noise(const float* src, float* buf, hipStream_t s);

  template <typename T> T* alloc(size_t n);
};

void set_error(const char* fmt, ...);
const char* get_error();

}
```

Baseline: 1.332 million.

## Fuse two-pass reductions via last-block tickets and fold loss copies into graphs

Replaces the two-kernel partial/final reduction pattern (colsum, LSTM colsums, D-head, MSE) with single kernels where the last block to finish, detected via an atomic ticket counter stored before the scratch buffer, performs the final sum. The D-head kernel also writes the fake loss directly, removing a separate copy. Loss copies to the caller buffer move inside the captured graph segments when the destination is stable. Together these aim to cut kernel launches and graph nodes per step, at the cost of threadfence/atomic overhead and extra graph variants keyed by the loss destination slot.

```diff
diff --git a/rsrgan_amd/csrc/kernels.h b/rsrgan_amd/csrc/kernels.h
--- a/rsrgan_amd/csrc/kernels.h
+++ b/rsrgan_amd/csrc/kernels.h
@@ -276,6 +276,7 @@
 void launch_gstate(const GStateArgs& a, hipStream_t s);
 struct ZeroList { int n; float* p[32]; unsigned len[32]; };
 void launch_zero_many(const ZeroList& zl, hipStream_t s);
+constexpr int RED_TICKETS = 4096;
 struct ColsumsBatch { const float* dz[4]; const float* cprev[4]; const float* ccur[4]; float* db[4]; float* dwi[4]; float* dwf[4]; float* dwo[4]; int n; };
 void launch_lstm_colsums_batch(const ColsumsBatch& bt, int rows, int H, float* scratch, hipStream_t s);
 void launch_lstm_colsums(const float* dz, const float* cprev, const float* ccur, float* db, float* dwi, float* dwf, float* dwo,
@@ -308,6 +309,7 @@
   float* logits; int ldl; float* dlogits; float* dout; int ldo; float* gw; float* gb;
   int T, Nd, n_real, dR; const float* t_real; const float* t_fake; float* loss3; float* part; int want_grads, want_wgrads;
   int Bp, Bt;
+  float* fake_out;
 };
 void launch_dhead(const DHeadArgs& a, hipStream_t s);
 void launch_lsgan(const float* logits, int ldl, float* dlogits, int T, int Nd, int n_real,
diff --git a/rsrgan_amd/csrc/kernels.hip b/rsrgan_amd/csrc/kernels.hip
--- a/rsrgan_amd/csrc/kernels.hip
+++ b/rsrgan_amd/csrc/kernels.hip
@@ -1,4 +1,5 @@
 #include <algorithm>
+#include <cstdio>
 #include <cstdlib>
 
 #include "kernels.h"
@@ -1319,9 +1320,28 @@
   hipLaunchKernelGGL(k_dropout_bwd, dim3((unsigned)std::min<size_t>((n + 255) / 256, 8192)), dim3(256), 0, s, y, d, rows, cols, ld, keep);
 }
 
+__device__ __forceinline__ bool red_last_block(unsigned* ticket, unsigned nblocks) {
+  __shared__ unsigned last;
+  __threadfence();
+  __syncthreads();
+  if (threadIdx.x == 0) {
+    const unsigned t = atomicAdd(ticket, 1u);
+    last = t == nblocks - 1 ? 1u : 0u;
+    if (last) *ticket = 0u;
+  }
+  __syncthreads();
+  const bool l = last != 0u;
+  if (l) __threadfence();
+  return l;
+}
+static inline unsigned* red_tickets(float* scratch, size_t n = 1) {
+  if (n > (size_t)RED_TICKETS) { fprintf(stderr, "rsrgan: a reduction of %zu column blocks exceeds its %d tickets\n", n, RED_TICKETS); abort(); }
+  return reinterpret_cast<unsigned*>(scratch) - RED_TICKETS;
+}
+
 constexpr int CS_SLICES = 64;
-__global__ __launch_bounds__(256) void k_colsum1(const float* __restrict__ a, int lda, const float* __restrict__ b, int ldb,
-                                                 float* __restrict__ scratch, int rows, int cols) {
+__global__ __launch_bounds__(256) void k_colsum(const float* __restrict__ a, int lda, const float* __restrict__ b, int ldb,
+                                                float* scratch, unsigned* tickets, float* __restrict__ out, int rows, int cols) {
   __shared__ float red[4][64];
   const int c = blockIdx.x * 64 + (threadIdx.x & 63), rl = threadIdx.x >> 6;
   const int per = (rows + CS_SLICES - 1) / CS_SLICES;
@@ -1337,13 +1357,12 @@
   __syncthreads();
   if (rl == 0 && c < cols)
     scratch[(size_t)blockIdx.y * cols + c] = ((red[0][threadIdx.x] + red[1][threadIdx.x]) + red[2][threadIdx.x]) + red[3][threadIdx.x];
-}
-__global__ void k_colsum2(const float* __restrict__ scratch, float* __restrict__ out, int cols) {
-  const int c = blockIdx.x * blockDim.x + threadIdx.x;
-  if (c >= cols) return;
-  float s = 0.f;
-  for (int i = 0; i < CS_SLICES; ++i) s += scratch[(size_t)i * cols + c];
-  out[c] = s;
+  if (!red_last_block(tickets + blockIdx.x, CS_SLICES)) return;
+  if (rl == 0 && c < cols) {
+    float t = 0.f;
+    for (int i = 0; i < CS_SLICES; ++i) t += scratch[(size_t)i * cols + c];
+    out[c] = t;
+  }
 }
 __global__ __launch_bounds__(256) void k_colsum1_n(const float* __restrict__ a, int lda, float* __restrict__ scratch, int rows, int cols,
                                                    int per) {
@@ -1381,8 +1400,19 @@
   hipLaunchKernelGGL(k_colsum2_n, dim3((cols + 63) / 64), dim3(256), 0, s, scratch, out, cols, slices);
 }
 
-__global__ __launch_bounds__(256) void k_lstm_colsums1(const float* __restrict__ dz, const float* __restrict__ cprev,
-                                                       const float* __restrict__ ccur, float* __restrict__ scratch, int rows, int H) {
+__device__ __forceinline__ void lstm_colsums_finish(const float* scratch, float* db, float* dwi, float* dwf, float* dwo, int H) {
+  const int c = blockIdx.x * 64 + (threadIdx.x & 63);
+  if (c >= H) return;
+  for (int k = threadIdx.x >> 6; k < 7; k += 4) {
+    float t = 0.f;
+#pragma unroll 8
+    for (int i = 0; i < CS_SLICES; ++i) t += scratch[((size_t)i * 7 + k) * H + c];
+    if (k < 4) db[k * H + c] = t;
+    else (k == 4 ? dwi : k == 5 ? dwf : dwo)[c] = t;
+  }
+}
+__device__ __forceinline__ void lstm_colsums_slice(const float* __restrict__ dz, const float* __restrict__ cprev,
+                                                   const float* __restrict__ ccur, float* scratch, int rows, int H) {
   __shared__ float red[7][4][64];
   const int c = blockIdx.x * 64 + (threadIdx.x & 63), rl = threadIdx.x >> 6;
   const int per = (rows + CS_SLICES - 1) / CS_SLICES;
@@ -1407,73 +1437,30 @@
       scratch[((size_t)blockIdx.y * 7 + k) * H + c] = ((red[k][0][x] + red[k][1][x]) + red[k][2][x]) + red[k][3][x];
   }
 }
-__global__ void k_lstm_colsums2(const float* __restrict__ scratch, float* __restrict__ db, float* __restrict__ dwi,
-                                float* __restrict__ dwf, float* __restrict__ dwo, int H) {
-  const int c = blockIdx.x * blockDim.x + threadIdx.x;
-  if (c >= H) return;
-  float s[7] = {0.f, 0.f, 0.f, 0.f, 0.f, 0.f, 0.f};
-#pragma unroll 8
-  for (int i = 0; i < CS_SLICES; ++i)
-#pragma unroll
-    for (int k = 0; k < 7; ++k) s[k] += scratch[((size_t)i * 7 + k) * H + c];
-  db[c] = s[0]; db[H + c] = s[1]; db[2 * H + c] = s[2]; db[3 * H + c] = s[3];
-  dwi[c] = s[4]; dwf[c] = s[5]; dwo[c] = s[6];
-}
-__global__ __launch_bounds__(256) void k_lstm_colsums1_b(const ColsumsBatch bt, float* __restrict__ scratch, int rows, int H) {
-  __shared__ float red[7][4][64];
+__global__ __launch_bounds__(256) void k_lstm_colsums(const float* __restrict__ dz, const float* __restrict__ cprev,
+                                                      const float* __restrict__ ccur, float* scratch, unsigned* tickets, float* db,
+                                                      float* dwi, float* dwf, float* dwo, int rows, int H) {
+  lstm_colsums_slice(dz, cprev, ccur, scratch, rows, H);
+  if (red_last_block(tickets + blockIdx.x, CS_SLICES)) lstm_colsums_finish(scratch, db, dwi, dwf, dwo, H);
+}
+__global__ __launch_bounds__(256) void k_lstm_colsums_b(const ColsumsBatch bt, float* scratch, unsigned* tickets, int rows, int H) {
   const int p = blockIdx.z;
-  const float* __restrict__ dz = bt.dz[p]; const float* __restrict__ cprev = bt.cprev[p]; const float* __restrict__ ccur = bt.ccur[p];
   scratch += (size_t)p * CS_SLICES * 7 * H;
-  const int c = blockIdx.x * 64 + (threadIdx.x & 63), rl = threadIdx.x >> 6;
-  const int per = (rows + CS_SLICES - 1) / CS_SLICES;
-  const int rbeg = blockIdx.y * per, rend = min(rows, rbeg + per);
-  float s[7] = {0.f, 0.f, 0.f, 0.f, 0.f, 0.f, 0.f};
-  if (c < H) {
-#pragma unroll 4
-    for (int r = rbeg + rl; r < rend; r += 4) {
-      const float* z = dz + (size_t)r * 4 * H + c;
-      const float di = z[0], dj = z[H], df = z[2 * H], d_o = z[3 * H];
-      const float cp = cprev[(size_t)r * H + c], cc = ccur[(size_t)r * H + c];
-      s[0] += di; s[1] += dj; s[2] += df; s[3] += d_o; s[4] += di * cp; s[5] += df * cp; s[6] += d_o * cc;
-    }
-  }
-#pragma unroll
-  for (int k = 0; k < 7; ++k) red[k][rl][threadIdx.x & 63] = s[k];
-  __syncthreads();
-  if (rl == 0 && c < H) {
-    const int x = threadIdx.x;
-#pragma unroll
-    for (int k = 0; k < 7; ++k)
-      scratch[((size_t)blockIdx.y * 7 + k) * H + c] = ((red[k][0][x] + red[k][1][x]) + red[k][2][x]) + red[k][3][x];
-  }
-}
-__global__ void k_lstm_colsums2_b(const float* __restrict__ scratch, const ColsumsBatch bt, int H) {
-  const int p = blockIdx.y;
-  scratch += (size_t)p * CS_SLICES * 7 * H;
-  const int c = blockIdx.x * blockDim.x + threadIdx.x;
-  if (c >= H) return;
-  float s[7] = {0.f, 0.f, 0.f, 0.f, 0.f, 0.f, 0.f};
-#pragma unroll 8
-  for (int i = 0; i < CS_SLICES; ++i)
-#pragma unroll
-    for (int k = 0; k < 7; ++k) s[k] += scratch[((size_t)i * 7 + k) * H + c];
-  float* db = bt.db[p];
-  db[c] = s[0]; db[H + c] = s[1]; db[2 * H + c] = s[2]; db[3 * H + c] = s[3];
-  bt.dwi[p][c] = s[4]; bt.dwf[p][c] = s[5]; bt.dwo[p][c] = s[6];
+  lstm_colsums_slice(bt.dz[p], bt.cprev[p], bt.ccur[p], scratch, rows, H);
+  if (red_last_block(tickets + p * gridDim.x + blockIdx.x, CS_SLICES)) lstm_colsums_finish(scratch, bt.db[p], bt.dwi[p], bt.dwf[p], bt.dwo[p], H);
 }
 void launch_lstm_colsums_batch(const ColsumsBatch& bt, int rows, int H, float* scratch, hipStream_t s) {
-  hipLaunchKernelGGL(k_lstm_colsums1_b, dim3((H + 63) / 64, CS_SLICES, bt.n), dim3(256), 0, s, bt, scratch, rows, H);
-  hipLaunchKernelGGL(k_lstm_colsums2_b, dim3((H + 255) / 256, bt.n), dim3(256), 0, s, scratch, bt, H);
+  hipLaunchKernelGGL(k_lstm_colsums_b, dim3((H + 63) / 64, CS_SLICES, bt.n), dim3(256), 0, s, bt, scratch, red_tickets(scratch, (size_t)bt.n * ((H + 63) / 64)), rows, H);
 }
 void launch_lstm_colsums(const float* dz, const float* cprev, const float* ccur, float* db, float* dwi, float* dwf, float* dwo,
                          int rows, int H, float* scratch, hipStream_t s) {
-  hipLaunchKernelGGL(k_lstm_colsums1, dim3((H + 63) / 64, CS_SLICES), dim3(256), 0, s, dz, cprev, ccur, scratch, rows, H);
-  hipLaunchKernelGGL(k_lstm_colsums2, dim3((H + 255) / 256), dim3(256), 0, s, scratch, db, dwi, dwf, dwo, H);
+  hipLaunchKernelGGL(k_lstm_colsums, dim3((H + 63) / 64, CS_SLICES), dim3(256), 0, s, dz, cprev, ccur, scratch, red_tickets(scratch, (H + 63) / 64), db,
+                     dwi, dwf, dwo, rows, H);
 }
 
 void launch_colsum(const float* a, int lda, const float* b, int ldb, float* out, int rows, int cols, float* scratch, hipStream_t s) {
-  hipLaunchKernelGGL(k_colsum1, dim3((cols + 63) / 64, CS_SLICES), dim3(256), 0, s, a, lda, b, ldb, scratch, rows, cols);
-  hipLaunchKernelGGL(k_colsum2, dim3((cols + 255) / 256), dim3(256), 0, s, scratch, out, cols);
+  hipLaunchKernelGGL(k_colsum, dim3((cols + 63) / 64, CS_SLICES), dim3(256), 0, s, a, lda, b, ldb, scratch, red_tickets(scratch, (cols + 63) / 64), out, rows,
+                     cols);
 }
 
 __device__ __forceinline__ float block_sum_1024(float v, float* red) {
@@ -1522,7 +1509,7 @@
                      clip_on ? 1 : 0, clip_lo, clip_hi, Bp, Bt);
 }
 
-__global__ __launch_bounds__(64) void k_dhead1(const DHeadArgs a) {
+__global__ __launch_bounds__(64) void k_dhead(const DHeadArgs a, unsigned* ticket) {
   __shared__ float wsh[DH_MAXR + 1];
   const int lane = threadIdx.x;
   const int rows = a.T * a.Nd, dR = a.dR;
@@ -1571,35 +1558,34 @@
     for (int c = 0; c < DH_MAXR; ++c)
       if (c < dR) { const float v = wsum(x[c] * dl); if (lane == 0) part[3 + c] = v; }
   }
-}
-__global__ __launch_bounds__(1024) void k_dhead2(const DHeadArgs a, int nblocks) {
-  __shared__ float tot[DH_MAXR + 3];
-  const int q = threadIdx.x >> 4, j = threadIdx.x & 15;
+  if (!red_last_block(ticket, gridDim.x)) return;
+  __shared__ float tot[2];
+  const int nblocks = gridDim.x, j = lane & 15;
   const int nq = a.want_wgrads ? 3 + a.dR : 2;
-  float s = 0.f;
-  if (q < nq)
-    for (int b = j; b < nblocks; b += 16) s += a.part[(size_t)b * (DH_MAXR + 3) + q];
-  s += __shfl_xor(s, 8); s += __shfl_xor(s, 4); s += __shfl_xor(s, 2); s += __shfl_xor(s, 1);
-  if (q < nq && j == 0) {
-    tot[q] = s;
-    if (a.want_wgrads) {
-      if (q == 2) a.gb[0] = s;
-      if (q >= 3) a.gw[(size_t)(q - 3) * a.ldw] = s;
-    }
-  }
-  __syncthreads();
-  if (threadIdx.x == 0) {
-    const int nr_ = a.Bp > 0 ? a.n_real / a.Bp * a.Bt : a.n_real, nf_ = a.Bp > 0 ? (a.Nd - a.n_real) / a.Bp * a.Bt : a.Nd - a.n_real;
-    const float cr = (float)a.T * (float)nr_, cf = (float)a.T * (float)nf_;
+  for (int q = lane >> 4; q < ((nq + 3) & ~3); q += 4) {
+    float s = 0.f;
+    if (q < nq)
+      for (int b = j; b < nblocks; b += 16) s += a.part[(size_t)b * (DH_MAXR + 3) + q];
+    s += __shfl_xor(s, 8); s += __shfl_xor(s, 4); s += __shfl_xor(s, 2); s += __shfl_xor(s, 1);
+    if (q < nq && j == 0) {
+      if (q < 2) tot[q] = s;
+      if (a.want_wgrads) {
+        if (q == 2) a.gb[0] = s;
+        if (q >= 3) a.gw[(size_t)(q - 3) * a.ldw] = s;
+      }
+    }
+  }
+  __syncthreads();
+  if (lane == 0) {
     const float lr_ = a.n_real > 0 ? tot[0] / cr : 0.f;
     const float lf_ = (a.Nd - a.n_real) > 0 ? tot[1] / cf : 0.f;
     a.loss3[0] = lr_; a.loss3[1] = lf_; a.loss3[2] = lr_ + lf_;
+    if (a.fake_out) *a.fake_out = lf_;
   }
 }
 void launch_dhead(const DHeadArgs& a, hipStream_t s) {
   const int rows = a.T * a.Nd, nb = (rows + 63) / 64;
-  hipLaunchKernelGGL(k_dhead1, dim3(nb), dim3(64), 0, s, a);
-  hipLaunchKernelGGL(k_dhead2, dim3(1), dim3(1024), 0, s, a, nb);
+  hipLaunchKernelGGL(k_dhead, dim3(nb), dim3(64), 0, s, a, red_tickets(a.part));
 }
 
 __global__ void k_build_joint(const float* __restrict__ x, int ldx, int off, int dim, const float* __restrict__ tail, int ldt, int Dt,
@@ -1631,9 +1617,9 @@
 }
 
 constexpr int MSE_BLOCKS = 256;
-__global__ __launch_bounds__(256) void k_mse1(const float* __restrict__ y, const float* __restrict__ lab, int ld,
-                                              float* __restrict__ dy, int rows, int D, const float* __restrict__ lambda,
-                                              int accumulate, float* __restrict__ scratch, int Bp, int Bt) {
+__global__ __launch_bounds__(256) void k_mse(const float* __restrict__ y, const float* __restrict__ lab, int ld,
+                                             float* __restrict__ dy, int rows, int D, const float* __restrict__ lambda,
+                                             int accumulate, float* scratch, unsigned* ticket, float* __restrict__ out, int Bp, int Bt) {
   __shared__ float red[16];
   const size_t total = (size_t)rows * D;
   const int rows_eff = Bp > 0 ? rows / Bp * Bt : rows;
@@ -1649,18 +1635,17 @@
   }
   s = block_sum_1024(s, red);
   if (threadIdx.x == 0) scratch[blockIdx.x] = s;
-}
-__global__ void k_mse2(const float* __restrict__ scratch, int rows, float* __restrict__ out) {
+  if (!red_last_block(ticket, MSE_BLOCKS)) return;
   if (threadIdx.x == 0) {
-    float s = 0.f;
-    for (int i = 0; i < MSE_BLOCKS; ++i) s += scratch[i];
-    *out = 0.5f * s / (float)rows;
+    float t = 0.f;
+    for (int i = 0; i < MSE_BLOCKS; ++i) t += scratch[i];
+    *out = 0.5f * t / (float)rows_eff;
   }
 }
 void launch_mse(const float* y, const float* lab, int ld, float* dy, int rows, int D, const float* lambda,
                 bool accumulate, float* loss_out, float* scratch, hipStream_t s, int Bp, int Bt) {
-  hipLaunchKernelGGL(k_mse1, dim3(MSE_BLOCKS), dim3(256), 0, s, y, lab, ld, dy, rows, D, lambda, accumulate ? 1 : 0, scratch, Bp, Bt);
-  hipLaunchKernelGGL(k_mse2, dim3(1), dim3(64), 0, s, scratch, Bp > 0 ? rows / Bp * Bt : rows, loss_out);
+  hipLaunchKernelGGL(k_mse, dim3(MSE_BLOCKS), dim3(256), 0, s, y, lab, ld, dy, rows, D, lambda, accumulate ? 1 : 0, scratch,
+                     red_tickets(scratch), loss_out, Bp, Bt);
 }
 
 __global__ void k_g_total(float* l4, const float* lambda) {
diff --git a/rsrgan_amd/csrc/model.cpp b/rsrgan_amd/csrc/model.cpp
--- a/rsrgan_amd/csrc/model.cpp
+++ b/rsrgan_amd/csrc/model.cpp
@@ -68,6 +68,14 @@
 void Model::drop_graphs() {
   for (auto& kv : graphs) if (kv.second.exec) (void)hipGraphExecDestroy(kv.second.exec);
   graphs.clear();
+}
+int Model::loss_slot(int kind, float* dst) {
+  if (!dst || !graphs_on()) return 0;
+  for (int i = 0; i < LOSS_DSTS; ++i) {
+    if (loss_dst[kind][i] == dst) return i + 1;
+    if (!loss_dst[kind][i]) { loss_dst[kind][i] = dst; return i + 1; }
+  }
+  return 0;
 }
 hipStream_t Model::enter(hipStream_t caller) {
   if (caller != nullptr || !main_s) return caller;
@@ -526,8 +534,10 @@
   maxcols = std::max(maxcols, (size_t)Din + 4);
   maxcols = std::max(maxcols, (size_t)std::max(ldP, ldDin));
   scratch_floats = std::max<size_t>(4 * 64 * maxcols, 16384);
-  scratch = alloc<float>(scratch_floats);
-  scratch2 = alloc<float>(std::max<size_t>(4 * 64 * maxcols, 1024));
+  scratch = alloc<float>(RED_TICKETS + scratch_floats);
+  scratch2 = alloc<float>(RED_TICKETS + std::max<size_t>(4 * 64 * maxcols, 1024));
+  if (scratch) scratch += RED_TICKETS;
+  if (scratch2) scratch2 += RED_TICKETS;
   g_fc_out_wT = g_dnn() ? nullptr : alloc<float>((size_t)Dout * ldP);
   if (hipStreamCreateWithFlags(&side, hipStreamNonBlocking) != hipSuccess) side = nullptr;
   if (hipEventCreateWithFlags(&ev_last, hipEventDisableTiming) != hipSuccess) ev_last = nullptr;
@@ -1660,7 +1670,7 @@
 }
 
 bool Model::d_head(int N, int T, int n_real, const float* t_real, const float* t_fake, float* loss3, bool want_grads, bool want_wgrads,
-                   hipStream_t s) {
+                   hipStream_t s, float* fake_out) {
   const int ldPd = pad4(dR), nb = (T * N + 63) / 64;
   if (!switches().dhead || d_dnn() || dl.empty() || dR % 4 != 0 || dR + 3 > 64 ||
       (size_t)nb * (DH_MAXR + 3) > scratch_floats) return false;
@@ -1669,7 +1679,7 @@
   a.logits = logits; a.ldl = 4; a.dlogits = dlogits; a.dout = d_dB; a.ldo = ldPd; a.gw = D.Gd(d_fc_w); a.gb = D.Gd(d_fc_b);
   a.T = T; a.Nd = N; a.n_real = n_real; a.dR = dR; a.t_real = t_real; a.t_fake = t_fake; a.loss3 = loss3; a.part = scratch;
   a.want_grads = want_grads ? 1 : 0; a.want_wgrads = want_wgrads ? 1 : 0;
-  a.Bp = pad_Bp(); a.Bt = Bt;
+  a.Bp = pad_Bp(); a.Bt = Bt; a.fake_out = fake_out;
   launch_dhead(a, s);
   return true;
 }
@@ -1757,7 +1767,8 @@
   }
   if (seq_drop_on()) launch_drop_tick(drop_ctr, s);
   const bool inl = fused_apply && switches().fused_seg && want_grads && !d_dnn() && graphs_on();
-  const unsigned kbits = (want_grads ? 1u : 0u) | (nr ? 2u : 0u) | (nf ? 4u : 0u) | (inl ? 8u : 0u) | (dsplit ? 16u : 0u);
+  const int lslot = loss_slot(0, out_losses);
+  const unsigned kbits = (want_grads ? 1u : 0u) | (nr ? 2u : 0u) | (nf ? 4u : 0u) | (inl ? 8u : 0u) | (dsplit ? 16u : 0u) | ((unsigned)lslot << 12);
   run_seg(seg_key(SEG_D, T, kbits), s, [&]() {
   if (!dsplit) launch_add_noise_rows(lab_tm, nr, xd, B, T, Dout, ldDout, 2 * B, 0, s);
   bool g_done = false;
@@ -1814,12 +1825,13 @@
     if (want_grads) d_backward_pass(2 * B, T, true, false, dlogits, s, head);
   }
   if (inl) apply_body(RSRGAN_NET_D, s);
+  if (lslot) launch_copy_f(losses, out_losses, 3, s);
   });
   d_partial_fresh = false;
   g_fwd_valid = true;
   if (inl) apply_inlined |= 2;
   if (want_grads) { finish_buckets(RSRGAN_NET_D, s); d_grads_ready = true; }
-  if (out_losses) launch_copy_f(losses, out_losses, 3, s);
+  if (out_losses && !lslot) launch_copy_f(losses, out_losses, 3, s);
   HIPC(hipGetLastError());
   return RSRGAN_OK;
 }
@@ -1901,6 +1913,8 @@
                           persist_backward_g(bw_chains[1], T, s, true);
   const bool inl = fused_apply && fused_seg && wave_bwd && !bucketed && graphs_on() && !(cfg.g_type == RSRGAN_G_LSTM && !fcs_inside);
   const unsigned kbits = (want_grads ? 1u : 0u) | (nf ? 2u : 0u) | (reuse ? 4u : 0u) | (l2_on ? 8u : 0u) | (bucketed ? 16u : 0u) | (inl ? 32u : 0u);
+  const int lslot = loss_slot(1, out_losses);
+  const unsigned lbits = (unsigned)lslot << 12;
   auto tail_body = [&]() {
     if (want_grads && l2_on) {
       launch_l2(G.w, G.g, G.ct, dyn + DYN_L2, G.partial, s);
@@ -1909,6 +1923,7 @@
       (void)hipMemsetAsync(losses + 5, 0, sizeof(float), s);
     }
     launch_g_total(losses + 3, dyn + DYN_LAMBDA, s);
+    if (lslot) launch_copy_f(losses + 3, out_losses, 4, s);
   };
 
   bool trail_plan = false;
@@ -1944,7 +1959,7 @@
     g_gemm_workers = saved_w;
     if (inl) { tail_body(); apply_body(RSRGAN_NET_G, s); }
   };
-  run_seg(seg_key(SEG_G_MAIN, T, kbits | (trail_plan ? 64u : 0u) | (gsplit ? 128u : 0u)), s, [&]() {
+  run_seg(seg_key(SEG_G_MAIN, T, kbits | (trail_plan ? 64u : 0u) | (gsplit ? 128u : 0u) | (inl && !gsplit ? lbits : 0u)), s, [&]() {
   if (trail_plan) gpersist_arm_bytes(g_dA, (size_t)T * B * ldP * sizeof(float), s);
   bool g_done = false;
   if (!reuse && !wavefront()) g_forward(T, s);
@@ -1985,13 +2000,13 @@
   if (d_dnn()) {
     d_dnn_forward_loss(T, B, 0, want_grads, tmp3, s);
   } else {
-    g_head = d_head(B, T, 0, dyn + DYN_D_REAL, dyn + DYN_D_REAL, tmp3, want_grads, false, s);
+    g_head = d_head(B, T, 0, dyn + DYN_D_REAL, dyn + DYN_D_REAL, tmp3, want_grads, false, s, losses + 3);
     if (!g_head) {
       d_logits(B, T, s);
       launch_lsgan(logits, 4, want_grads ? dlogits : nullptr, T, B, 0, dyn + DYN_D_REAL, dyn + DYN_D_REAL, tmp3, s, false, 0.f, 0.f, pad_Bp(), Bt);
     }
   }
-  launch_copy_f(tmp3 + 1, losses + 3, 1, s);
+  if (!g_head) launch_copy_f(tmp3 + 1, losses + 3, 1, s);
   if (want_grads && d_dnn()) {
     float* dyd = fc_backward(D, dfc, d_act, T * B, dlogits, false, true, s);
     launch_mse(y_tm, lab_tm, ldDout, dyd, T * B, Dout, dyn + DYN_LAMBDA, true, losses + 4, scratch, s, pad_Bp(), Bt);
@@ -2057,7 +2072,7 @@
     defer_wgrads = false;
     (void)hipEventRecord(ev_dfree, s);
     dfree_inside = true; dfree_current = true;
-    run_seg(seg_key(SEG_G_MAIN, T, kbits | 64u | 256u), s, bwd_rest);
+    run_seg(seg_key(SEG_G_MAIN, T, kbits | 64u | 256u | (inl ? lbits : 0u)), s, bwd_rest);
   }
   if (inl) apply_inlined |= 1;
   if (!reuse) g_fwd_valid = true;
@@ -2084,13 +2099,13 @@
       }
     }
   }
-  if (!inl) run_seg(seg_key(SEG_G_TAIL, T, kbits), s, tail_body);
+  if (!inl) run_seg(seg_key(SEG_G_TAIL, T, kbits | lbits), s, tail_body);
   if (want_grads) {
     if (l2_on) for (auto& bk : gbk[RSRGAN_NET_G]) bk.marked = false;
     finish_buckets(RSRGAN_NET_G, s);
     g_grads_ready = true;
   }
-  if (out_losses) launch_copy_f(losses + 3, out_losses, 4, s);
+  if (out_losses && !lslot) launch_copy_f(losses + 3, out_losses, 4, s);
   HIPC(hipGetLastError());
   return RSRGAN_OK;
 }
diff --git a/rsrgan_amd/csrc/model.h b/rsrgan_amd/csrc/model.h
--- a/rsrgan_amd/csrc/model.h
+++ b/rsrgan_amd/csrc/model.h
@@ -280,7 +280,7 @@
   void g_forward_tail(int T, hipStream_t s);
   void d_logits(int N, int T, hipStream_t s);
   void d_backward_pass(int N, int T, bool want_wgrads, bool need_dx0, const float* dlog, hipStream_t s, bool head_done = false);
-  bool d_head(int N, int T, int n_real, const float* t_real, const float* t_fake, float* loss3, bool want_grads, bool want_wgrads, hipStream_t s);
+  bool d_head(int N, int T, int n_real, const float* t_real, const float* t_fake, float* loss3, bool want_grads, bool want_wgrads, hipStream_t s, float* fake_out = nullptr);
   void g_backward_pass(int T, float* dy, hipStream_t s);
   int d_backward(const float* x, const float* labels, const int32_t* lengths, int T, const float* nr, const float* nf,
                  float* out_losses, bool want_grads, hipStream_t s);
@@ -357,6 +357,9 @@
   bool graphs_on() const { return (cfg.flags & RSRGAN_FLAG_GRAPH) != 0 && wavefront() && !overlap() && !prof_on && !g_dnn() && sw.graphs; }
   template <class F> void run_seg(uint64_t key, hipStream_t s, F&& body);
   void drop_graphs();
+  static constexpr int LOSS_DSTS = 4;
+  float* loss_dst[2][LOSS_DSTS] = {};
+  int loss_slot(int kind, float* dst);
   hipStream_t enter(hipStream_t caller);
   void leave(hipStream_t caller, hipStream_t work);
   const float* stage_noise(const float* src, float* buf, hipStream_t s);
```

Result: slower. 1.218 million (-8.5%).
